# alex-petrenko/sample-factory

Measured on AMD Instinct MI355X. Metric: env-steps/sec (whole node), 4096 envs, 84x84x4 obs, higher is better.
Workload: dtype f32

## Files before the change

include/sf_hip.h:

```cpp
#ifndef SF_HIP_H
#define SF_HIP_H

#include <stdint.h>

#ifdef __cplusplus
extern "C" {
#endif

#define SF_OK 0
#define SF_ERR_ARG (-1)
#define SF_ERR_LAUNCH (-2)
#define SF_ERR_UNSUPPORTED (-3)
#define SF_MAX_ACTION_HEADS 64

const char *sf_last_error(void);
int sf_abi_version(void);

int sf_valid_mask(const int32_t *policy_id, const float *policy_version, uint8_t *valids, uint8_t *valids_flat,
                  float *actions, int num_actions, float *log_prob_actions, int E, int T, int my_policy_id,
                  int train_step, int max_policy_lag, int32_t *num_invalid, void *stream);

int sf_gae_returns(float *rewards, const uint8_t *dones, const uint8_t *time_outs, const float *values,
                   const uint8_t *valids, const double *rms_stats, int E, int T, float gamma, float gae_lambda,
                   int value_bootstrap, float *advantages, float *returns, void *stream);
// ... 35 lines not shown
    int32_t action_kind;
    int32_t dense_adv;
    int32_t num_heads;
    int32_t head_n[8];
    int32_t old_values_T;
} sf_loss_cfg;

int sf_ppo_loss(const float *params, int ld_params, const float *values, int ld_values, const float *actions,
                const float *old_logp, const float *old_params, const float *old_values, const float *adv,
                const float *targets, const uint8_t *valids, const int32_t *index, int64_t offset, int64_t n, int A,
                const sf_loss_cfg *h_cfg, const double *moments, double *sums, float *g_params, float *g_values,
                float *ratio_out ,
                void *stream);
int sf_ppo_loss_heads(const float *params, int ld_params, const float *values, int ld_values, const float *actions,
                      const float *old_logp, const float *old_params, const float *old_values, const float *adv,
                      const float *targets, const uint8_t *valids, const int32_t *index, int64_t offset, int64_t n, int A,
                      const sf_loss_cfg *h_cfg, const double *moments, double *sums, float *g_params, float *g_values,
                      float *ratio_out, const int32_t *head_n , int num_heads, void *stream);
int sf_ppo_loss_masked(const float *params, int ld_params, const float *values, int ld_values, const float *actions,
                       const float *old_logp, const float *old_params, const float *old_values, const float *adv,
                       const float *targets, const uint8_t *valids, const int32_t *index, int64_t offset, int64_t n, int A,
                       const sf_loss_cfg *h_cfg, const double *moments, double *sums, float *g_params, float *g_values,
                       float *ratio_out, const int32_t *head_n , int num_heads, const uint8_t *mask,
                       int64_t ld_mask, int mask_T, void *stream);
int sf_vtrace_masked(const float *params, int ld_params, const float *values, int ld_values, const float *actions,
                     const float *old_logp, const float *rewards, const uint8_t *dones, const int32_t *index,
                     int64_t offset, int64_t n, int A, int action_kind, int recurrence, float gamma, float rho_hat,
                     float c_hat, float *vs, float *adv, const int32_t *head_n , int num_heads,
                     const uint8_t *mask, int64_t ld_mask, int mask_T, void *stream);
int sf_consistency_loss(const float *params_t, const float *params_s, int ld_params, const float *values_t,
                        const float *values_s, int ld_values, const uint8_t *valids, const int32_t *index, int64_t offset,
                        int64_t n, int A, int action_kind, const int32_t *head_n , int num_heads,
                        float coeff_policy, float coeff_value, const double *moments, double *sums, float *g_params_s,
                        float *g_values_s, void *stream);
int sf_loss_scalars(const double *sums, const double *moments, const sf_loss_cfg *h_cfg, float *out, void *stream);
int sf_train_summaries(const uint8_t *valids, const float *ratio, const float *values, int ld_values,
                       const float *old_values, int old_values_T, const float *actions, int num_actions, const float *adv,
                       int dense_adv, const int32_t *policy_id, const float *policy_version, const float *action_logits,
                       int A, const int32_t *index, int64_t offset, int64_t n, int my_policy_id, int train_step,
                       float clip_ratio, const float *exp_avg_sq, int64_t P, double *out, void *stream);

int sf_minibatch_indices(int32_t *out, int64_t experience_size, int recurrence, int shuffle, uint32_t seed,
                         uint32_t epoch, void *stream);
int sf_minibatch_expand(const int32_t *chunk_starts, int32_t *out, int64_t experience_size, int recurrence,
                        void *stream);

int sf_grad_sumsq(const float *g, int64_t P, double *sumsq, void *stream);
int sf_adam_step(float *p, const float *g, float *m, float *v, int64_t P, int step, float lr, float beta1,
                 float beta2, float eps, float max_grad_norm, const double *sumsq, float grad_scale,
                 const uint32_t *skip_flag, void *stream);
int sf_adam_step_dlr(float *p, const float *g, float *m, float *v, int64_t P, int step, const float *lr_dev,
                     float lr_scale, float beta1, float beta2, float eps, float max_grad_norm, const double *sumsq,
                     float grad_scale, const uint32_t *skip_flag, void *stream);
int sf_lr_kl_adaptive(const float *kl, float *lr_dev, float threshold, float lr_min, float lr_max, float *lr_out,
                      void *stream);
int sf_clock_probe(unsigned long long *out, int spin_cycles, void *stream);

int sf_lamb_step(float *p, const float *g, float *m, float *v, float *scratch, const uint8_t *seg_id, double *seg_sums,
                 int64_t P, int num_segments, int step, float lr, float beta1, float beta2, float eps,
                 float weight_decay, float min_trust, float max_grad_norm, const double *sumsq, float grad_scale,
                 const uint32_t *skip_flag, void *stream);

int sf_sample_write_step(const float *logits, int ld_logits, const float *values, int ld_values, int B, int A, int T,
                         int t, uint32_t seed, uint32_t step, uint32_t row0, float policy_version, int deterministic,
                         int action_kind, float *traj_actions,
                         float *traj_logits, float *traj_logp, float *traj_values, float *traj_policy_version,
                         int32_t *env_actions, void *stream);

int sf_sample_write_step_masked(const float *logits, int ld_logits, const float *values, int ld_values,
                                const uint8_t *action_mask, int64_t ld_mask, int B, int A, int T, int t, uint32_t seed,
                                uint32_t step, uint32_t row0, float policy_version, int deterministic,
                                float *traj_actions, float *traj_logits, float *traj_logp, float *traj_values,
                                float *traj_policy_version, int32_t *env_actions, void *stream);

int sf_sample_write_step_tuple(const float *logits, int ld_logits, const float *values, int ld_values, int B,
                               int num_heads, const int32_t *head_n, int T, int t, uint32_t seed, uint32_t step,
                               uint32_t row0, float policy_version, int deterministic, float *traj_actions,
                               float *traj_logits, float *traj_logp, float *traj_values, float *traj_policy_version,
                               int32_t *env_actions, void *stream);

int sf_sample_write_step_tuple_masked(const float *logits, int ld_logits, const float *values, int ld_values,
                                      const uint8_t *action_mask, int64_t ld_mask, int B, int num_heads,
                                      const int32_t *head_n, int T, int t, uint32_t seed, uint32_t step, uint32_t row0,
                                      float policy_version, int deterministic, float *traj_actions, float *traj_logits,
                                      float *traj_logp, float *traj_values, float *traj_policy_version,
                                      int32_t *env_actions, void *stream);

int sf_traj_write_env_step(const float *rewards, const uint8_t *terminated, const uint8_t *truncated, int B, int T,
                           int t, float reward_scale, float reward_clip, int policy_id, float *traj_rewards,
                           uint8_t *traj_dones, uint8_t *traj_time_outs, int32_t *traj_policy_id, float *ep_return,
                           int32_t *ep_len, double *ep_stats, void *stream);

int sf_traj_write_env_step_active(const float *rewards, const uint8_t *terminated, const uint8_t *truncated, int B, int T,
                                  int t, float reward_scale, float reward_clip, int policy_id, float *traj_rewards,
                                  uint8_t *traj_dones, uint8_t *traj_time_outs, int32_t *traj_policy_id, float *ep_return,
                                  int32_t *ep_len, double *ep_stats, const uint8_t *active_in, uint8_t *active_state,
                                  void *stream);

int sf_synth_vec_step(float *state, const float *actions, int64_t act_stride, float *obs_out, int64_t out_stride, int B,
                      int D, int A, int env0, uint32_t seed, uint32_t step, int reset, float *rewards,
                      uint8_t *terminated, void *stream);

int sf_h2d_rows(void *dst, int64_t dst_pitch, const void *src, int64_t src_pitch, int64_t row_bytes, int64_t rows,
                void *stream);
int sf_copy_rows(void *dst, int64_t dst_pitch, const void *src, int64_t src_pitch, int64_t row_bytes, int64_t rows,
                 void *stream);
// ... 12 lines not shown
                 void *stream);
int sf_synth_step(const int32_t *actions, int B, int env0, int num_actions, uint32_t seed, uint32_t step,
                  float *rewards, uint8_t *terminated, void *stream);

int sf_pixcatch_state_words(int k);
int sf_pixcatch_reset(int32_t *state, uint8_t *obs_out, int64_t out_pitch, int N, int env0, uint32_t seed, int H, int W,
                      int k, int balls, void *stream);
int sf_pixcatch_step(int32_t *state, const int32_t *actions, uint8_t *obs_out, int64_t out_pitch, float *rewards,
                     uint8_t *terminated, int N, int env0, uint32_t seed, int H, int W, int k, int balls, void *stream);
int sf_pixcatch_reset_levels(int32_t *state, uint8_t *obs_out, int64_t out_pitch, int N, int env0, uint32_t seed, int H,
                             int W, int k, int balls, int decoys, int levels, uint32_t start_level, void *stream);
int sf_pixcatch_step_levels(int32_t *state, const int32_t *actions, uint8_t *obs_out, int64_t out_pitch, float *rewards,
                            uint8_t *terminated, int N, int env0, uint32_t seed, int H, int W, int k, int balls, int decoys,
                            int levels, uint32_t start_level, void *stream);

int sf_random_shift_gather(void *dst, int64_t dst_sample_pitch, const void *src, int64_t src_sample_pitch,
                           const int32_t *index, int64_t offset, int64_t n, int traj_T, int C, int H, int W, int elem_bytes,
                           int pad, int recurrence, uint32_t seed, uint32_t draw_id, void *stream);

typedef struct {
    int32_t Cin, H, W;
    int32_t Cout, KH, KW, stride;
    int32_t OH, OW;
    int32_t in_u8;
    int32_t relu;
    int32_t traj_T;
    float sub_mean, inv_scale;
} sf_conv_desc;

int64_t sf_conv_fwd_workspace(int64_t n, const sf_conv_desc *h_desc);
int sf_conv_fwd(const void *in, int64_t in_sample_stride, const int32_t *index, int64_t offset, const float *w,
                const float *bias, float *out, int64_t n, const sf_conv_desc *h_desc, void *workspace,
                int64_t workspace_bytes, void *stream);
int64_t sf_conv_wgrad_workspace(int64_t n, const sf_conv_desc *h_desc);
int sf_conv_wgrad(const void *in, int64_t in_sample_stride, const int32_t *index, int64_t offset, const float *dout,
                  float *dw, float *db, int64_t n, const sf_conv_desc *h_desc, void *workspace, void *stream);
int sf_conv_dgrad(const float *dout, const float *w, const float *in_act, float *din, int64_t n,
                  const sf_conv_desc *h_desc, void *stream);
int sf_conv_relu_mask_supported(int64_t n, const sf_conv_desc *h_desc);
int sf_conv_fwd_relu_mask(const void *in, int64_t in_sample_stride, const int32_t *index, int64_t offset, const float *w,
                          const float *bias, float *out, uint32_t *relu_mask, int64_t n, const sf_conv_desc *h_desc,
                          void *stream);
int sf_conv_wgrad_relu_mask(const void *in, int64_t in_sample_stride, const int32_t *index, int64_t offset,
                            const float *dout, const uint32_t *relu_mask, float *dw, float *db, int64_t n,
                            const sf_conv_desc *h_desc, void *workspace, void *stream);

int sf_conv_norm_supported(int64_t n, const sf_conv_desc *h_desc);
int sf_conv_fwd_norm(const void *in, int64_t in_sample_stride, const int32_t *index, int64_t offset, const float *mu,
                     const float *rstd, const float *w, const float *bias, float *out, int64_t n,
                     const sf_conv_desc *h_desc, void *stream);
int sf_conv_wgrad_norm(const void *in, int64_t in_sample_stride, const int32_t *index, int64_t offset, const float *mu,
                       const float *rstd, const float *dout, float *dw, float *db, int64_t n, const sf_conv_desc *h_desc,
                       void *workspace, void *stream);

int sf_mlp2_fwd(const float *x, int64_t x_stride, int64_t n, int D, float sub_mean, float inv_scale, const float *mu,
                const float *rstd, const float *w1, const float *b1, int H1, const float *w2, const float *b2, int H2,
                int act, float *out, void *stream);

int sf_rnn_store_state(const float *h, const float *c, const uint8_t *dones, int64_t done_stride, float *out,
                       int64_t out_stride, int64_t B, int H, void *stream);

int sf_rnn_store_state_held(const float *h, const float *c, const uint8_t *dones, int64_t done_stride, const float *prev,
                            int64_t prev_stride, const int32_t *policy_id, int64_t pid_stride, float *out,
                            int64_t out_stride, int64_t B, int H, void *stream);

int sf_rnn_chunk_setup(const uint8_t *dones, const uint8_t *valids, const float *rnn_states, const int32_t *index,
                       int64_t offset, int Cn, int R, int S, int traj_T, float *keep_tm, float *h0, void *stream);

int sf_lstm_seq_supported(int Cn, int H);
int sf_lstm_seq_fwd(const float *gx, const float *whh, const float *bhh, const float *keep, float *gates, float *hprev,
                    float *hout, float *cprev, float *cout, uint32_t *sync, int R, int Cn, int H, int env_major,
                    void *stream);
int sf_lstm_seq_bwd(const float *dout, const float *gates, const float *cprev, const float *cout, const float *keep,
                    const float *whh, float *dgx, uint32_t *sync, int R, int Cn, int H, int env_major, void *stream);

int sf_gru_seq_fwd(const float *gx, const float *whh, const float *bhh, const float *keep, float *gates, float *hprev,
                   float *hout, uint32_t *sync, int R, int Cn, int H, int env_major, void *stream);
int sf_gru_seq_bwd(const float *dout, const float *gates, const float *hprev, const float *keep, const float *whh,
                   float *dgx, float *dgh, uint32_t *sync, int R, int Cn, int H, int env_major, void *stream);

int sf_seq_fwd_x_supported(int Cn, int H, int Kx);
int sf_lstm_seq_fwd_x(const float *x, const float *wih_t, const float *bih, int Kx, const float *whh, const float *bhh,
                      const float *keep, float *gates, float *hprev, float *hout, float *cprev, float *cout,
                      uint32_t *sync, int R, int Cn, int H, int env_major, void *stream);
int sf_gru_seq_fwd_x(const float *x, const float *wih_t, const float *bih, int Kx, const float *whh, const float *bhh,
                     const float *keep, float *gates, float *hprev, float *hout, uint32_t *sync, int R, int Cn, int H,
                     int env_major, void *stream);

int sf_rnn_rowseq_supported(int kind, int Cn, int H);
int sf_rnn_rowseq_fwd(int kind, const float *gx, const float *whh, const float *bhh, const float *keep, float *gates,
                      float *hprev, float *hout, float *cprev, float *cout, int R, int Cn, int H, int env_major, void *stream);
int sf_rnn_rowseq_bwd(int kind, const float *dout, const float *gates, const float *hprev, const float *cprev,
                      const float *cout, const float *keep, const float *whh, float *dgx, float *dgh,
                      int R, int Cn, int H, int env_major, void *stream);

int sf_rnn_wideseq_supported(int kind, int Cn, int H);
int sf_rnn_seq_slab_rows(int kind, int H, int pass);
int sf_rnn_wideseq_fwd(int kind, const float *gx, const float *whh, const float *bhh, const float *keep, float *gates,
                       float *hprev, float *hout, float *cprev, float *cout, uint32_t *sync, int R, int Cn, int H,
                       int env_major, void *stream);
int sf_rnn_wideseq_bwd(int kind, const float *dout, const float *gates, const float *hprev, const float *cprev,
                       const float *cout, const float *keep, const float *whh, float *dgx, float *dgh, uint32_t *sync,
                       int R, int Cn, int H, int env_major, void *stream);

#define SF_DP_UNIQUE_ID_BYTES 128
int sf_dp_unique_id(void *out_id);
// ... 88 lines not shown
```

sample_factory_amd/algo/learning/learner.py:

```python
from __future__ import annotations

import glob
import time
import os
from os.path import join
from typing import Dict, List, Optional, Tuple

import numpy as np
import torch

from sample_factory_amd import lib
from sample_factory_amd.algo.learning.dp import ReplicaGroup
from sample_factory_amd.algo.utils.tensor_dict import TensorDict
from sample_factory_amd.cfg.arguments import augment_consistency_coeff
from sample_factory_amd.envs.frame_ops import random_shift_seed
from sample_factory_amd.envs.spaces import (action_head_sizes, calc_num_action_parameters, calc_num_actions, is_box,
                                             is_discrete)
from sample_factory_amd.model.actor_critic import ActorCritic
from sample_factory_amd.model.model_factory import create_actor_critic
from sample_factory_amd.utils.attr_dict import AttrDict
from sample_factory_amd.utils.decay import LinearDecay
from sample_factory_amd.utils.utils import log

LEARNER_ENV_STEPS, POLICY_ID_KEY, STATS_KEY, TRAIN_STATS = "learner_env_steps", "policy_id", "stats", "train"
# ... 308 lines not shown
        ac = self.actor_critic
        keep_p = ac.flat_params.clone()
        sd = dict(ref)
        ac.load_state_dict(sd, strict=False)
        flat.copy_(ac.flat_params)
        ac.flat_params.copy_(keep_p)
        ac.params_changed()

    def load_from_checkpoint(self, policy_id, load_progress=True) -> None:
        prefix = dict(latest="checkpoint", best="best")[self.cfg.load_checkpoint_kind]
        cps = self.get_checkpoints(self.checkpoint_dir(self.cfg, policy_id), pattern=f"{prefix}_*")
        cp = self.load_checkpoint(cps, self.device)
        if cp is not None:
            self._load_state(cp, load_progress)

    def set_new_cfg(self, new_cfg: Dict) -> None:
        self.new_cfg = new_cfg

    def set_policy_to_load(self, policy_to_load) -> None:
        self.policy_to_load = policy_to_load

    def _refresh_loss_cfg(self) -> None:
        cfg = self.cfg
        self.loss_cfg = lib.sf_loss_cfg(
            clip_ratio=cfg.ppo_clip_ratio, clip_value=cfg.ppo_clip_value, value_loss_coeff=cfg.value_loss_coeff,
            exploration_coeff=cfg.exploration_loss_coeff, kl_coeff=cfg.kl_loss_coeff,
            exploration_kind=0 if cfg.exploration_loss_coeff == 0.0 else (1 if cfg.exploration_loss == "entropy" else 2),
            action_kind=1 if is_box(self.env_info.action_space) else 0, dense_adv=int(bool(cfg.with_vtrace)))
        heads = action_head_sizes(self.env_info.action_space)
        self._head_sizes = heads
        if 1 < len(heads) <= len(self.loss_cfg.head_n):
            self.loss_cfg.num_heads = len(heads)
            for i, nh in enumerate(heads):
                self.loss_cfg.head_n[i] = nh

    def _maybe_update_cfg(self) -> None:
        if self.new_cfg is None:
            return
        for key, value in self.new_cfg.items():
            setattr(self.cfg, key, value)
        if self.cfg.lr_schedule == "constant" and self.curr_lr != self.cfg.learning_rate:
            self.curr_lr = self.cfg.learning_rate
        self._refresh_loss_cfg()
        self.new_cfg = None

    def _maybe_load_policy(self) -> None:
        if self.policy_to_load is None:
            return
        self.load_from_checkpoint(self.policy_to_load, load_progress=False)
        self.train_step += self.cfg.max_policy_lag + 1
        self.policy_versions_tensor[self.policy_id] = self.train_step
        self.policy_to_load = None

    def _prepare_batch(self, batch: TensorDict) -> Tuple[AttrDict, int, int]:
        cfg, ac = self.cfg, self.actor_critic
        multi = getattr(ac, "multi_key", False)
        obs = {k: batch["obs"][k] for k in ac.obs_keys} if multi else batch["obs"]["obs"]
        E, T = batch["rewards"].shape
        N = E * T
        valids_flat = ac._buf(("prep", "valids_flat"), (N,), dtype=torch.bool)
        lib.valid_mask(batch["policy_id"], batch["policy_version"], batch["valids"], batch["actions"],
                       self.num_actions, batch["log_prob_actions"], self.policy_id, self.train_step,
                       cfg.max_policy_lag, self._num_invalid, valids_flat=valids_flat)
        if not ac.training:
            ac.train()
        if ac.obs_normalizer is not None:
            ac.obs_normalizer.update(obs, ac.obs_elems, E * (T + 1))
        last = {k: v[:, T] for k, v in obs.items()} if multi else obs[:, T]
        rnn = dict(states=batch["rnn_states"][:, T]) if cfg.use_rnn else None
        heads = ac.forward_heads(last, E, sample_stride=0 if multi else obs.stride(0), tag="boot", rnn=rnn)[-1]
        lib.copy_rows(batch["values"][:, T], heads[:, 0])
        adv = torch.empty((E, T), dtype=torch.float32, device=self.device)
        ret = torch.empty((E, T), dtype=torch.float32, device=self.device)
        buff = AttrDict()
        if not cfg.with_vtrace:
            rms = ac.returns_normalizer.stats if cfg.normalize_returns else None
            lib.gae_returns(batch["rewards"], batch["dones"], batch["time_outs"], batch["values"], batch["valids"],
                            rms, cfg.gamma, cfg.gae_lambda, cfg.value_bootstrap, adv, ret)
            buff.advantages, buff.returns = adv.view(N), ret.view(N)
        elif cfg.value_bootstrap:
            lib.gae_returns(batch["rewards"], batch["dones"], batch["time_outs"], batch["values"], batch["valids"],
                            None, cfg.gamma, cfg.gae_lambda, True, adv, ret)
        buff.obs = obs
        buff.actions = batch["actions"].view(N, self.num_actions)
        buff.action_logits = batch["action_logits"].view(N, self.num_action_params)
        buff.log_prob_actions = batch["log_prob_actions"].view(N)
        buff.rewards = batch["rewards"].view(N)
        buff.dones = batch["dones"].view(N)
        buff.policy_id, buff.policy_version = batch["policy_id"].view(N), batch["policy_version"].view(N)
        if cfg.use_rnn:
            buff.rnn_states = batch["rnn_states"]
        buff["values"] = batch["values"]
        buff.valids = valids_flat
        buff.E, buff.T = E, T
        if getattr(self, "_loss_mask_on", False):
            buff.action_mask = batch["obs"]["action_mask"]
        if cfg.normalize_returns and not cfg.with_vtrace:
            ac.returns_normalizer(buff.returns)
        num_invalids = int(self._num_invalid.item())
        if self.dp:
            t = torch.tensor([num_invalids], dtype=torch.int64, device=self.device)
            self._all_reduce(t)
            self._global_invalids = int(t.item())
        else:
            self._global_invalids = num_invalids
        return buff, N, num_invalids

    def _get_minibatches(self, batch_size, experience_size):
        cfg = self.cfg
        assert cfg.rollout % cfg.recurrence == 0
        assert experience_size % batch_size == 0, f"experience size: {experience_size}, batch size: {batch_size}"
        n_mb = cfg.num_batches_per_epoch
        if n_mb == 1:
            return [(None, 0, experience_size)]
        assert n_mb * batch_size == experience_size, \
            f"dataset of {experience_size} samples != num_batches_per_epoch {n_mb} x batch_size {batch_size}"
        if cfg.shuffle_minibatches:
            idx = torch.empty(experience_size, dtype=torch.int32, device=self.device)
            if getattr(cfg, "device_shuffle", False):
                seed = (cfg.seed or 0) * 7919 + self.policy_id
                lib.minibatch_indices(idx, experience_size, cfg.recurrence, True, seed, self._shuffle_epoch)
                self._shuffle_epoch += 1
            else:
                starts = np.random.permutation(np.arange(0, experience_size, cfg.recurrence))
                starts_dev = torch.from_numpy(starts.astype(np.int32)).to(self.device, non_blocking=True)
                lib.minibatch_expand(starts_dev, idx, experience_size, cfg.recurrence)
            return [(idx[i * batch_size:(i + 1) * batch_size], 0, batch_size) for i in range(experience_size // batch_size)]
        return [(None, i * batch_size, batch_size) for i in range(n_mb)]

    _shuffle_epoch = 0

    def _calculate_losses(self, mb: AttrDict, num_invalids: int):
        from sample_factory_amd.algo.utils.action_distributions import get_action_distribution
        buff, part = (mb if isinstance(mb, tuple) else (mb, None))
        if part is None:
            part = (None, 0, buff.E * buff.T)
        acts, g_heads, sc = self._losses_native(buff, part, num_invalids)
        index, offset, n = part
        heads = acts[-1]
        A = self.num_action_params
        space = self.env_info.action_space
        rows = index.long() if index is not None else torch.arange(offset, offset + n, device=self.device)
        mask = buff.get("action_mask")
        mrows = None if mask is None else mask[:, :buff.T].reshape(buff.E * buff.T, -1)[rows]
        dist = get_action_distribution(space, heads[:n, 1:1 + A], mrows)
        dist.raw_logits, dist.values = heads[:n, 1:1 + A], heads[:n, 0]
        kl_old = dist.kl_divergence(get_action_distribution(space, buff.action_logits[rows], mrows))[buff.valids[rows]]
        summaries = AttrDict(adv_mean=sc[6], adv_std=sc[7], num_valid=sc[8], entropy=sc[9], kl_divergence_max=sc[5],
                             kl_old_mean=sc[4].clone(), ratio=self._ratio[:n], values=heads[:n, 0], g_heads=g_heads)
        return dist, sc[0].clone(), sc[1].clone(), kl_old, sc[2].clone(), sc[3].clone(), summaries

    def _losses_native(self, buff: AttrDict, mb, num_invalids: int, scalars_out: Optional[torch.Tensor] = None,
                       moments: Optional[torch.Tensor] = None, first_of: Optional[Tuple[int, int]] = None):
        cfg, ac = self.cfg, self.actor_critic
        index, offset, n = mb
        A = self.num_action_params
        alpha = getattr(self, "_cons_coeff", 0.0) if getattr(self, "_shift_pad", 0) > 0 else 0.0
        m = 2 * n if alpha > 0.0 else n
        rnn = None
# ... 37 lines not shown
            vs = ac._buf(("vt", "vs"), (n,))
            adv = ac._buf(("vt", "adv"), (n,))
            lib.vtrace(params, ld, values, ld, buff.actions, buff.log_prob_actions, buff.rewards, buff.dones, index,
                       offset, n, A, self.loss_cfg.action_kind, cfg.recurrence, cfg.gamma, cfg.vtrace_rho,
                       cfg.vtrace_c, vs, adv, head_sizes=self._head_sizes, **mkw)
            lib.moments(adv, buff.valids, index, n, self._moments, offset=offset, dense_x=True)
            adv_arr, tgt_arr = adv, vs
        elif moments is None:
            lib.moments(buff.advantages, buff.valids, index, n, self._moments, offset=offset)
            adv_arr, tgt_arr = buff.advantages, buff.returns
        else:
            adv_arr, tgt_arr = buff.advantages, buff.returns
        if moments is None:
            moments = self._moments
            self._all_reduce(moments)
        self._ratio = ac._buf(("loss", "ratio"), (n,))
        self.loss_cfg.old_values_T = buff.T
        lib.ppo_loss(params, ld, values, ld, buff.actions, buff.log_prob_actions, buff.action_logits, buff["values"],
                     adv_arr, tgt_arr, buff.valids, index, offset, n, A, self.loss_cfg, moments, self._sums,
                     g_heads[:n, 1:], g_heads[:n, 0], ratio_out=self._ratio, head_sizes=self._head_sizes, **mkw)
        if m > n:
            if not hasattr(self, "_cons_sums"):
                self._cons_sums = torch.zeros(4, dtype=torch.float64, device=self.device)
            lib.consistency_loss(params, heads[n:, 1:], ld, values, heads[n:, 0], ld, buff.valids, index, offset, n, A,
                                 self.loss_cfg.action_kind, alpha, alpha, moments, self._cons_sums, g_heads[n:, 1:],
                                 g_heads[n:, 0], head_sizes=self._head_sizes)
        self._last_mb = (index, offset, n, values, adv_arr)
        if self.dp and self._dp_reduce_each_mb:
            self.group.loss_sums(self._sums)
        out = scalars_out if scalars_out is not None else torch.zeros(16, dtype=torch.float32, device=self.device)
        lib.loss_scalars(self._sums, moments, self.loss_cfg, out)
        if m > n:
            c = self._cons_sums
            nv = c[3].clamp(min=1.0)
            out[11:14].copy_(torch.stack((c[0] / nv, c[2], c[1] / nv)))
        return acts, g_heads, out

    def _epoch_moments(self, buff: AttrDict, minibatches) -> Optional[torch.Tensor]:
        if not self.dp or self.cfg.with_vtrace or not getattr(self.cfg, "dp_epoch_moments", True):
            return None
        tab = self.actor_critic._buf(("loss", "epoch_moments"), (len(minibatches), 3), dtype=torch.float64)
        for i, (index, offset, n) in enumerate(minibatches):
            lib.moments(buff.advantages, buff.valids, index, n, tab[i], offset=offset)
        self._all_reduce(tab)
        return tab

    def _train(self, buff: AttrDict, batch_size: int, experience_size: int, num_invalids: int) -> Optional[AttrDict]:
        cfg, ac = self.cfg, self.actor_critic
        early_stopping_tolerance = 1e-6
        prev_epoch_actor_loss = 1e9
        recent_kls: List[float] = []
        num_sgd_steps = 0
        n_mb = cfg.num_batches_per_epoch
        self._scalars = ac._buf(("loss", "scalars"), (cfg.num_epochs * n_mb, 16))
        global_size = experience_size * self.world
        need_kl_each_mb = self.lr_scheduler.invoke_after_each_minibatch() and isinstance(self.lr_scheduler, KlAdaptiveScheduler)
        self._dp_reduce_each_mb = need_kl_each_mb
        lr_on_device = need_kl_each_mb and cfg.optimizer == "adam"
        if lr_on_device:
            if not hasattr(self, "_lr_dev"):
                self._lr_dev = torch.zeros(1, dtype=torch.float32, device=self.device)
            self._lr_dev.fill_(float(self.curr_lr))
        self._grad_norms = []
        skip = ac.rnn_abort_word() if hasattr(ac, "rnn_abort_word") else None
        if skip is not None:
            ac.rnn_abort_clear()
        for epoch in range(cfg.num_epochs):
            minibatches = self._get_minibatches(batch_size, experience_size)
            mom_tab = self._epoch_moments(buff, minibatches)
            for batch_num, mb in enumerate(minibatches):
                row = self._scalars[epoch * n_mb + batch_num]
                acts, g_heads, _ = self._losses_native(buff, mb, num_invalids, row,
                                                       moments=None if mom_tab is None else mom_tab[batch_num],
                                                       first_of=(epoch, batch_num))
                index, offset, n = mb
                if self._dp_split is not None:
                    cut = ac._segs[self._dp_split][0]
                    pending = []
                    ac.backward(acts, g_heads, self._mb_frames[0], self._mb_rows, sample_stride=ac.obs_elems,
                                **self._mb_frames[1],
                                on_layer_done=lambda li: pending.append(self.group.all_reduce_grads_async(
                                    ac.flat_grads[cut:])) if li == self._dp_split else None)
                    self.group.all_reduce_grads(ac.flat_grads[:cut])
                    for work in pending:
                        work.wait()
                else:
                    ac.backward(acts, g_heads, self._mb_frames[0], self._mb_rows, sample_stride=ac.obs_elems,
                                **self._mb_frames[1])
                    if self.dp:
                        self.group.all_reduce_grads(ac.flat_grads)
                actual_lr = self.curr_lr
                valid_frac = 1.0
                if self._global_invalids > 0:
                    valid_frac = (global_size - self._global_invalids) / global_size
                    actual_lr = self.curr_lr * valid_frac
                self.adam_step_count += 1
                use_clip = cfg.max_grad_norm > 0.0
                if use_clip or getattr(cfg, "record_grad_norm", False):
                    lib.grad_sumsq(ac.flat_grads, self._sumsq)
                    if getattr(cfg, "record_grad_norm", False):
                        self._grad_norms.append(float(self._sumsq.sqrt().item()))
                if cfg.optimizer == "lamb":
                    if self._lamb is None:
                        seg, nseg = ac.tensor_segment_ids()
                        self._lamb = (seg, nseg, torch.empty_like(ac.flat_params),
                                      torch.zeros(128, dtype=torch.float64, device=self.device))
                    seg, nseg, scratch, seg_sums = self._lamb
                    lib.lamb_step(ac.flat_params, ac.flat_grads, self.exp_avg, self.exp_avg_sq, scratch, seg, seg_sums,
                                  nseg, self.adam_step_count, actual_lr, cfg.adam_beta1, cfg.adam_beta2, cfg.adam_eps,
                                  1e-4, 0.01, cfg.max_grad_norm if use_clip else 0.0, self._sumsq if use_clip else None,
                                  skip_flag=skip)
                elif lr_on_device:
                    lib.adam_step_dlr(ac.flat_params, ac.flat_grads, self.exp_avg, self.exp_avg_sq, self.adam_step_count,
                                      self._lr_dev, valid_frac, cfg.adam_beta1, cfg.adam_beta2, cfg.adam_eps,
                                      cfg.max_grad_norm if use_clip else 0.0, self._sumsq if use_clip else None,
                                      skip_flag=skip)
                else:
                    lib.adam_step(ac.flat_params, ac.flat_grads, self.exp_avg, self.exp_avg_sq, self.adam_step_count,
                                  actual_lr, cfg.adam_beta1, cfg.adam_beta2, cfg.adam_eps,
                                  cfg.max_grad_norm if use_clip else 0.0, self._sumsq if use_clip else None,
                                  skip_flag=skip)
                ac.params_changed()
                num_sgd_steps += 1
                self.train_step += 1
                if lr_on_device:
                    sch = self.lr_scheduler
                    lib.lr_kl_adaptive(row[4:5], self._lr_dev, sch.threshold, sch.min_lr, sch.max_lr, lr_out=row[10:11])
                elif need_kl_each_mb:
                    recent_kls.append(float(row[4].item()))
                    self.curr_lr = self.lr_scheduler.update(self.curr_lr, recent_kls)
                elif self.lr_scheduler.invoke_after_each_minibatch():
                    self.curr_lr = self.lr_scheduler.update(self.curr_lr, recent_kls)
                self.policy_versions_tensor[self.policy_id] = self.train_step
            blk = self._scalars[epoch * n_mb:(epoch + 1) * n_mb]
            if self.dp and not need_kl_each_mb:
                flag = (skip.to(torch.float32) if skip is not None else blk.new_zeros(1)).expand(blk.shape[0], 1)
                pack = torch.cat([blk[:, [0, 1, 2, 3, 4, 9, 5]], flag], dim=1).contiguous()
                self.group.reduce_sum_max(pack, (6, 7))
                blk[:, [0, 1, 2, 3, 4, 9, 5]] = pack[:, :7]
                aborted = skip is not None and bool(pack[0, 7].item() != 0)
            elif self.dp and skip is not None:
                aborted = bool(self.group.all_reduce_max(skip.to(torch.float32)).item() != 0)
            else:
                aborted = skip is not None and ac.rnn_pass_aborted()
            rows = blk.cpu()
            if aborted:
                raise lib.SfHipError(
                    "a fused recurrent sequence pass was aborted (a work-group never arrived: is the GPU shared with "
                    "another process?); the optimiser steps after it were skipped, the weights are those of the last "
                    "good SGD step; set SF_LSTM_SEQ=0 to use the per-step kernels")
            actor_losses = (rows[:, 0] + rows[:, 1] + rows[:, 2]).double().numpy()
            if lr_on_device:
                self.curr_lr = float(rows[-1, 10])
                actual_lr = self.curr_lr * valid_frac
            if not need_kl_each_mb or lr_on_device:
                recent_kls.extend(rows[:, 4].double().tolist())
            if self.lr_scheduler.invoke_after_each_epoch():
                self.curr_lr = self.lr_scheduler.update(self.curr_lr, recent_kls)
            new_epoch_actor_loss = float(np.mean(actor_losses))
            if abs(prev_epoch_actor_loss - new_epoch_actor_loss) < early_stopping_tolerance:
                break
            prev_epoch_actor_loss = new_epoch_actor_loss
        last = rows[-1]
        stats = AttrDict(lr=self.curr_lr, actual_lr=actual_lr, env_steps=self.env_steps,
                         policy_loss=float(last[0]), exploration_loss=float(last[1]),
                         kl_loss=float(last[2]), value_loss=float(last[3]), kl_divergence=float(last[4]),
                         kl_divergence_max=float(last[5]), adv_mean=float(last[6]), adv_std=float(last[7]),
                         entropy=float(last[9]), loss=float(last[0] + last[1] + last[2] + last[3]),
                         num_sgd_steps=num_sgd_steps)
        if getattr(self, "_cons_coeff", 0.0) > 0.0:
            stats.update(consistency_kl=float(last[11]), consistency_kl_max=float(last[12]),
                         consistency_value=float(last[13]))
        if self._should_save_summaries():
            stats.update(self._record_summaries(buff))
            self._last_summary_time = time.time()
        self.last_summary = stats
        return stats

    _last_summary_time = 0.0
    _summary_rate_decay = LinearDecay([(0, 2.0), (100000, 60.0), (1000000, 120.0)])

    def _should_save_summaries(self) -> bool:
        every = self._summary_rate_decay.at(float(self.train_step))
        return time.time() - self._last_summary_time >= every or getattr(self.cfg, "summaries_every_train", False)

    def _record_summaries(self, buff: AttrDict) -> Dict[str, float]:
        index, offset, n, values, adv_arr = self._last_mb
        if not hasattr(self, "_summ"):
            self._summ = torch.empty(24, dtype=torch.float64, device=self.device)
        ld = values.stride(0) if values.dim() == 1 else 1
        lib.train_summaries(buff.valids, self._ratio, values, ld, buff["values"], buff.T, buff.actions, self.num_actions,
                            adv_arr, bool(self.cfg.with_vtrace), buff.policy_id, buff.policy_version, buff.action_logits,
                            self.num_action_params, index, offset, n, self.policy_id, self.train_step,
                            self.loss_cfg.clip_ratio, self.exp_avg_sq, self._summ)
        o = self._summ.cpu().tolist()
        rows, nv, ns = o[0], o[1], o[2]
        has_v, has_s = nv > 0, ns > 0
        return dict(
            valids_fraction=nv / rows, same_policy_fraction=ns / rows, value=o[3] / rows,
            ratio_mean=o[4] / nv if has_v else 0.0, ratio_min=o[8] if has_v else 1.0, ratio_max=o[9] if has_v else 1.0,
            fraction_clipped=o[5] / nv if has_v else 0.0, value_delta=o[6] / rows, value_delta_max=o[10],
            act_min=o[11], act_max=o[12], adv_min=o[13], adv_max=o[14], max_abs_logprob=o[15],
            version_diff_avg=o[7] / ns if has_s else 0.0, version_diff_min=o[16] if has_s else 0.0,
            version_diff_max=o[17] if has_s else 0.0, grad_norm=float(self._sumsq.sqrt().item()),
            adam_max_second_moment=o[18])

    def train(self, batch: TensorDict) -> Optional[Dict]:
        self._maybe_update_cfg()
        self._maybe_load_policy()
        buff, experience_size, num_invalids = self._prepare_batch(batch)
        if self._global_invalids >= experience_size * self.world:
            return None
        train_stats = self._train(buff, self.cfg.batch_size, experience_size, num_invalids)
        frameskip = self.env_info.frameskip if self.cfg.summaries_use_frameskip else 1
        self.env_steps += experience_size * self.world * frameskip
        stats = {LEARNER_ENV_STEPS: self.env_steps, POLICY_ID_KEY: self.policy_id}
        if train_stats is not None:
            stats[TRAIN_STATS] = train_stats
        return stats
```

sample_factory_amd/csrc/sf_nn.hip:

```cpp
#include "sf_common.h"
#include <stdarg.h>
#include <stdlib.h>
#include <string.h>
#ifndef SF_GLDS_ABLATE
#define SF_GLDS_ABLATE 0
#endif
#include <type_traits>
#include <algorithm>

#define STREAM(s) reinterpret_cast<hipStream_t>(s)

typedef float f32x16 __attribute__((ext_vector_type(16)));

extern "C" int sf_selftest_host(void) {
    const uint32_t ds[] = {1, 2, 3, 4, 6, 7, 9, 20, 32, 33, 49, 64, 81, 84, 128, 400, 512, 576, 3136, 7056, 28224, 65535, 1000003};
    for (uint32_t d : ds) {
        const FastDiv f = make_fastdiv(d);
        const uint32_t ns[] = {0, 1, d - 1, d, d + 1, 2 * d - 1, 2 * d, 12345678, 0x7FFFFFFFu, 0x7FFFFFFFu - d, 13107200, 13107199};
        for (uint32_t n : ns) if (fdiv(n, f) != n / d) return -1;
        for (uint32_t n = 0; n < 200000; n += 7) if (fdiv(n, f) != n / d) return -2;
        for (uint32_t n = 0x7FFFFFFFu; n > 0x7FFFFFFFu - 100000; n -= 13) if (fdiv(n, f) != n / d) return -3;
    }
    const uint32_t areas[] = {1, 2, 3, 35, 70, 96, 485, 5760, 19200, 33600, 76800, 921600, 8388607, 8388608};
    for (uint32_t D : areas) {
// ... 554 lines not shown
                const int64_t base = patch_base(m, mok, po);
                if constexpr (MODE == MODE_F32)
                    ra[s].v = *reinterpret_cast<const float4 *>(reinterpret_cast<const float *>(in) + base + tapo[s]);
                else
                    ra[s] = load_act_raw<MODE_GENERIC>(g, in, base, po, (uint32_t)(k0row + kg[s]), aok[s]);
            }
        }
#pragma unroll
        for (int s = 0; s < T::SB; ++s) {
            const int64_t m = mc + bkk0 + s * BROWS;
            bok[s] = m < mend;
            rb[s] = load_row_raw<VECB>(dy, bok[s] ? m : mbeg, n0 + bcg, N);
        }
    };
    const bool do_colsum = partial_b != nullptr && blockIdx.x == 0 && tid < BN;
    float colacc = 0.f;
    if (mbeg < mend) gload(mbeg);
    for (int64_t mc = mbeg; mc < mend; mc += 32) {
        __syncthreads();
#pragma unroll
        for (int s = 0; s < T::SA; ++s) {
            const int lrow = FR ? (tid & 31) : (tid >> 5) + 8 * s;
            *reinterpret_cast<float4 *>(&As[lrow * LDA + kg[s]]) =
                act_finish<MODE>(g, ra[s], MODE != MODE_GENERIC || aok[s]);
        }
        const bool tail = mc + 32 > mend;
#pragma unroll
        for (int s = 0; s < T::SB; ++s)
            *reinterpret_cast<float4 *>(&Bs[(bkk0 + s * BROWS) * LDB + bcg]) =
                (VECB && !tail) ? rb[s] : row_finish(rb[s], bok[s], n0 + bcg, N);
        __syncthreads();
        if (mc + 32 < mend) gload(mc + 32);
        if (do_colsum) {
#pragma unroll 8
            for (int kk = 0; kk < 32; ++kk) colacc += Bs[kk * LDB + tid];
        }
        mma_chunk<T::TM, T::TN, LDA, LDB>(As, Bs, wm * T::TM * 32, wn * T::TN * 32, lane, acc);
    }
    if (do_colsum && n0 + tid < N) partial_b[(int64_t)blockIdx.z * N + n0 + tid] = colacc;
    float *dst = partial + (int64_t)blockIdx.z * K * N;
#pragma unroll
    for (int tm = 0; tm < T::TM; ++tm)
#pragma unroll
        for (int tn = 0; tn < T::TN; ++tn) {
            const int n = n0 + wn * T::TN * 32 + tn * 32 + (lane & 31);
#pragma unroll
            for (int r = 0; r < 16; ++r) {
                const int k = k0row + wm * T::TM * 32 + tm * 32 + FRAG_ROW(r, lane);
                if (k < K && n < N) dst[(int64_t)k * N + n] = acc[tm][tn][r];
            }
        }
}

__global__ __launch_bounds__(256) void k_reduce_partials(const float *__restrict__ partial, float *__restrict__ out,
                                                         int64_t n, int Z) {
    for (int64_t i = (int64_t)blockIdx.x * blockDim.x + threadIdx.x; i < n; i += (int64_t)gridDim.x * blockDim.x) {
        float s[8] = {0.f, 0.f, 0.f, 0.f, 0.f, 0.f, 0.f, 0.f};
        int z = 0;
        for (; z + 8 <= Z; z += 8) {
#pragma unroll
            for (int j = 0; j < 8; ++j) s[j] += partial[(int64_t)(z + j) * n + i];
        }
        for (int j = 0; z < Z; ++z, ++j) s[j] += partial[(int64_t)z * n + i];
        out[i] = ((s[0] + s[1]) + (s[2] + s[3])) + ((s[4] + s[5]) + (s[6] + s[7]));
    }
}

__global__ __launch_bounds__(256) void k_reduce_partials_tree(const float *__restrict__ partial, float *__restrict__ out,
                                                              int64_t n, int Z) {
    __shared__ float sm[8][33];
    const int li = threadIdx.x & 31, zg = threadIdx.x >> 5;
    const int64_t i = (int64_t)blockIdx.x * 32 + li;
    const int zper = (Z + 7) / 8, z0 = zg * zper, z1 = z0 + zper < Z ? z0 + zper : Z;
    float s[8] = {0.f, 0.f, 0.f, 0.f, 0.f, 0.f, 0.f, 0.f};
    if (i < n) {
        int z = z0;
        for (; z + 8 <= z1; z += 8) {
#pragma unroll
            for (int j = 0; j < 8; ++j) s[j] += partial[(int64_t)(z + j) * n + i];
        }
        for (int j = 0; z < z1; ++z, ++j) s[j] += partial[(int64_t)z * n + i];
    }
    sm[zg][li] = ((s[0] + s[1]) + (s[2] + s[3])) + ((s[4] + s[5]) + (s[6] + s[7]));
    __syncthreads();
    if (zg == 0 && i < n)
        out[i] = ((sm[0][li] + sm[1][li]) + (sm[2][li] + sm[3][li])) + ((sm[4][li] + sm[5][li]) + (sm[6][li] + sm[7][li]));
}
#define SF_SWITCHES(X)                                                                                                  \
    X(reduce_tree, "SF_REDUCE_TREE", 1) X(conv1_bf16, "SF_CONV1_BF16", 1) X(conv1_img, "SF_CONV1_IMG", 1)              \
    X(conv1_wgs, "SF_CONV1_WGS", 2) X(conv1_wide, "SF_CONV1_WIDE", 1) X(conv1_norm, "SF_CONV1_NORM", 1)                \
    X(relu_mask, "SF_RELU_MASK", 1) X(fwd_img, "SF_FWD_IMG", 1) X(linear_narrow, "SF_LINEAR_NARROW", 1)                \
    X(linear_dual, "SF_LINEAR_DUAL", 1) X(glds_cfg, "SF_GLDS_CFG", 0) X(glds_splitk, "SF_GLDS_SPLITK", 1)              \
    X(glds_fc64, "SF_GLDS_FC64", 1) X(glds_wide_min, "SF_GLDS_WIDE_MIN", 384) X(glds_min_tiles, "SF_GLDS_MIN_TILES", 768) \
    X(glds_small64, "SF_GLDS_SMALL64", 256) X(glds_force64, "SF_GLDS_FORCE64", 0) X(glds_split64, "SF_GLDS_SPLIT64", 32) \
    X(glds_zl, "SF_GLDS_ZL", 2) X(glds_tailsplit, "SF_GLDS_TAILSPLIT", 1) X(glds_tall, "SF_GLDS_TALL", 0)              \
    X(glds_persist, "SF_GLDS_PERSIST", 0) X(xcd_raster, "SF_XCD_RASTER", 1) X(xcd_rows, "SF_XCD_ROWS", 0)              \
    X(tap_perm, "SF_TAP_PERM", 0) X(wgrad_glds, "SF_WGRAD_GLDS", 1) X(wgrad_glds_min, "SF_WGRAD_GLDS_MIN", -1)         \
    X(wgrad_glds_k64, "SF_WGRAD_GLDS_K64", 1) X(wgrad_img, "SF_WGRAD_IMG", 3) X(wgrad_zl, "SF_WGRAD_ZL", 1)            \
    X(dgrad_linear, "SF_DGRAD_LINEAR", 1) X(dgrad_linear64, "SF_DGRAD_LINEAR64", 1) X(dgrad_lpt, "SF_DGRAD_LPT", 1)    \
    X(dgrad_zl, "SF_DGRAD_ZL", 3) X(dgrad_pix, "SF_DGRAD_PIX", 1) X(debug_occ, "SF_DEBUG_OCC", 0)
struct Switches {
#define X(field, name, dflt) int64_t field;
    SF_SWITCHES(X)
#undef X
    bool debug_img;
};
static int64_t env_num(const char *name, int64_t dflt) {
    const char *v = getenv(name);
    return v ? atoll(v) : dflt;
}
static Switches read_switches() {
    Switches s;
#define X(field, name, dflt) s.field = env_num(name, dflt);
    SF_SWITCHES(X)
#undef X
    s.debug_img = getenv("SF_DEBUG_IMG") != nullptr;
    return s;
}
static const Switches &sw() {
    static const Switches s = read_switches();
    return s;
}

static void launch_reduce_partials(const float *partial, float *out, int64_t n, int Z, hipStream_t st) {
    if (sw().reduce_tree && Z >= 64 && (n + 255) / 256 < 256)
        k_reduce_partials_tree<<<dim3((unsigned)((n + 31) / 32)), dim3(256), 0, st>>>(partial, out, n, Z);
    else
        k_reduce_partials<<<dim3((unsigned)((n + 255) / 256 < 2048 ? (n + 255) / 256 : 2048)), dim3(256), 0, st>>>(partial, out, n, Z);
}

template <int BM, int BN, int WM, int WN, bool VEC>
__global__ __launch_bounds__(256) void k_conv_dgrad(ConvG g, const float *__restrict__ dy,
                                                    const float *__restrict__ w, const float *__restrict__ in_act,
                                                    float *__restrict__ din, int64_t nsamples) {
    using T = Tile<BM, BN, WM, WN>;
    constexpr int LDA = BM + 1, LDB = BN + 1;
    __shared__ __attribute__((aligned(16))) float As[32 * LDA];
    __shared__ __attribute__((aligned(16))) float Bs[32 * LDB];
    const int tid = threadIdx.x, lane = tid & 63, wave = tid >> 6;
    const int wm = wave / WN, wn = wave % WN;
    const int ph = blockIdx.z / g.S, pw = blockIdx.z % g.S;
    const int Hc = (g.H - ph + g.S - 1) / g.S, Wc = (g.W - pw + g.S - 1) / g.S;
    const int KHs = (g.KH - ph + g.S - 1) / g.S, KWs = (g.KW - pw + g.S - 1) / g.S;
    const int64_t Mc = nsamples * Hc * Wc;
    const int64_t m0 = (int64_t)blockIdx.x * BM;
    if (m0 >= Mc || Hc <= 0 || Wc <= 0) return;
    const int n0 = blockIdx.y * BN;
    const int Cin = g.Cin, Cout = g.Cout;
    const int Kp = KHs * KWs * Cout;

    const int kq = (tid & 7) * 4;
    const FastDiv fHW = g.dHcWc[blockIdx.z], fW = g.dWc[blockIdx.z], fKWs = g.dKWs[blockIdx.z];
    int arow[T::SA], aih[T::SA], aiw[T::SA];
    bool aval[T::SA];
    const uint32_t HcWc = (uint32_t)(Hc * Wc);
#pragma unroll
    for (int s = 0; s < T::SA; ++s) {
        const int64_t m = m0 + (tid >> 3) + 32 * s;
        aval[s] = m < Mc;
        const uint32_t mm = aval[s] ? (uint32_t)m : 0u;
        const uint32_t smp = fdiv(mm, fHW), pix = mm - smp * HcWc;
        aih[s] = (int)fdiv(pix, fW);
        aiw[s] = (int)pix - aih[s] * Wc;
        arow[s] = (int)(smp * (uint32_t)(g.OH * g.OW)) + aih[s] * g.OW + aiw[s];
    }
    const bool kfull = (Kp & 31) == 0;
    f32x16 acc[T::TM][T::TN];
    ZERO_ACC(acc);

    float4 ra[T::SA], rb[T::SB];
    bool aok[T::SA], bok = true;
    int ncol = 0;
    auto gload = [&](int k0) {
        const int k = k0 + kq;
        const bool kval = k < Kp;
        const int kc = kval ? k : 0;
        const int tap = (int)fdiv((uint32_t)kc, g.dCout);
        const int n = kc - tap * Cout;
        ncol = n;
        const int a = (int)fdiv((uint32_t)tap, fKWs), b = tap - a * KWs;
        const int drow = a * g.OW + b;
// ... 687 lines not shown
extern "C" int sf_conv_fwd_t_os2(const float *in, int64_t in_sample_stride, const float *in2, const float *wt, const float *bias,
                                 float *out, int64_t out_sample_stride, float *out2, int64_t keep_n, int64_t n,
                                 const sf_conv_desc *h_desc, void *stream) {
    return conv_fwd_t_os_impl("sf_conv_fwd_t_os2", in, in_sample_stride, in2, wt, bias, out, out_sample_stride, out2, keep_n, n,
                              h_desc, stream);
}
static int conv_fwd_os_supported_impl(int op, int64_t n, int64_t keep_n, const sf_conv_desc *h_desc, int64_t in_sample_stride,
                                      int64_t out_sample_stride) {
    if (!h_desc || n <= 0 || keep_n < 0 || keep_n > n || check_desc(h_desc, "sf_conv_fwd_os_supported") != 0 ||
        in_sample_stride % 4 != 0 || !out_stride_ok(h_desc, nullptr, out_sample_stride) ||
        n * (int64_t)h_desc->OH * h_desc->OW >= (1LL << 31))
        return 0;
    if (op == 0) {
        if (!relu_mask_ok(h_desc, n)) return 0;
        Operands o = query_operands(h_desc, false);
        o.stride = in_sample_stride;
        return plan_conv_fwd(h_desc, make_geom(h_desc), n, o).kernel == K_CONV1_U8_BF16_W ? 1 : 0;
    }
    if (op != 3) return 0;
    const ConvPlan p = plan_conv_fwd_t(h_desc, n, in_sample_stride, nullptr, true, keep_n);
    return (p.kernel == K_FWD_IMG || p.kernel == K_FWD_GLDS_ZT || p.kernel == K_FWD_GLDS_Z) && p.splits == 1 ? 1 : 0;
}
extern "C" int sf_conv_fwd_os_supported(int op, int64_t n, const sf_conv_desc *h_desc, int64_t in_sample_stride,
                                        int64_t out_sample_stride) {
    return conv_fwd_os_supported_impl(op, n, n, h_desc, in_sample_stride, out_sample_stride);
}
extern "C" int sf_conv_fwd_os2_supported(int op, int64_t n, int64_t keep_n, const sf_conv_desc *h_desc, int64_t in_sample_stride,
                                         int64_t out_sample_stride) {
    return conv_fwd_os_supported_impl(op, n, keep_n, h_desc, in_sample_stride, out_sample_stride);
}

extern "C" int sf_linear_fwd_dual_supported(int64_t n, int N, int K1, int K2) {
    return sw().linear_dual && n > 0 && N >= 64 && K1 > 0 && K2 > 0 && K1 % 32 == 0 && K2 % 32 == 0 && n < (1LL << 31) &&
           cdiv64(n, 128) * (int64_t)cdiv64(N, 64) >= 256;
}
extern "C" int sf_linear_fwd_dual(const float *a1, int64_t lda1, const float *w1t, const float *bias1, int K1,
                                  const float *a2, int64_t lda2, const float *w2t, const float *bias2, int K2, float *out,
                                  int64_t n, int N, int gru_H, void *stream) {
    SF_REQUIRE(a1 && w1t && a2 && w2t && out && n > 0 && N > 0, "sf_linear_fwd_dual: bad args");
    SF_REQUIRE(K1 > 0 && K2 > 0 && K1 % 32 == 0 && K2 % 32 == 0 && lda1 % 4 == 0 && lda2 % 4 == 0 && n < (1LL << 31),
               "sf_linear_fwd_dual: K1, K2 must be multiples of 32 and the row strides multiples of 4 (K1=%d K2=%d)", K1, K2);
    SF_REQUIRE((((uintptr_t)a1 | (uintptr_t)a2 | (uintptr_t)w1t | (uintptr_t)w2t) & 15) == 0,
               "sf_linear_fwd_dual: operands must be 16-byte aligned");
    SF_REQUIRE(gru_H == 0 || (gru_H > 0 && gru_H % 64 == 0 && N == 4 * gru_H),
               "sf_linear_fwd_dual: the GRU column layout needs N == 4 * gru_H and gru_H %% 64 == 0 (N=%d gru_H=%d)", N, gru_H);
    k_fwd_glds2<128, 64, 2, 2><<<dim3(cdiv64(n, 128), cdiv64(N, 64)), dim3(256), 0, STREAM(stream)>>>(
        a1, lda1, w1t, bias1, K1, a2, lda2, w2t, bias2, K2, out, n, N, gru_H);
    return sf_launch_status("sf_linear_fwd_dual");
}
extern "C" int sf_transpose(const float *w, float *wt, int K, int N, void *stream) {
    SF_REQUIRE(w && wt && K > 0 && N > 0, "sf_transpose: bad args");
    k_transpose<<<dim3(cdiv64(K, 32), cdiv64(N, 32)), dim3(256), 0, STREAM(stream)>>>(w, wt, K, N);
    return sf_launch_status("sf_transpose");
}

struct SplitPlan {
    int Z;
    int64_t m_per_split;
};
static SplitPlan plan_splits(int64_t Mtot, int K, int N, int BM, int BN, int bpc = 0) {
    const int64_t tiles = (int64_t)((K + BM - 1) / BM) * ((N + BN - 1) / BN);
    const int64_t chunks = (Mtot + 31) / 32;
    int64_t zcap = (2304 + tiles - 1) / tiles;
    const int64_t zmax = (chunks + 7) / 8;
    if (zcap > zmax) zcap = zmax;
    if (zcap < 1) zcap = 1;
    if (zcap > 1024) zcap = 1024;
    int64_t Z = zcap;
    if (bpc > 0) {
        const double slots = 256.0 * bpc;
        double best = -1.0;
        for (int64_t z = 1; z <= zcap; ++z) {
            const double u = (double)(tiles * z) / slots, rounds = u <= 1.0 ? 1.0 : (double)(int64_t)(u + 0.999999);
            double eff = u / rounds;
            if (tiles * z < 256) eff *= 0.5;
            if (eff > best + 0.02) { best = eff; Z = z; }
        }
    }
    SplitPlan p;
    p.m_per_split = ((chunks + Z - 1) / Z) * 32;
    p.Z = (int)((Mtot + p.m_per_split - 1) / p.m_per_split);
    return p;
}
template <int BK, int BN, int WM, int WN>
static int occ_wgrad_glds() {
    static const int v = occupancy_of(k_wgrad_glds<BK, BN, WM, WN>);
    return v;
}
static inline int wgrad_bn(int N) { return N <= 32 ? 32 : 64; }
static int wgrad_ws_partials(int64_t Mtot, int K, int N) { return plan_splits(Mtot, K, N, 128, wgrad_bn(N)).Z; }
struct WgradGlds {
    int cfg;
    int BK, BN, Z;
    int64_t m_per_split;
};
static WgradGlds plan_wgrad_glds(int64_t Mtot, int K, int N, bool query_occupancy = false) {
    WgradGlds q;
    const bool k256 = K >= 256 && (K + 255) / 256 * 256 <= (K + 127) / 128 * 128;
    q.cfg = N >= 128 ? 1 : (k256 ? 0 : 2);
    if (sw().wgrad_glds >= 2) q.cfg = sw().wgrad_glds - 2;
    if (K == 64 && N >= 128) q.cfg = 3;
    q.BK = q.cfg == 0 ? 256 : q.cfg == 3 ? 64 : 128;
    q.BN = (q.cfg == 1 || q.cfg == 3) ? 128 : 64;
    int bpc = 0;
    if (query_occupancy)
        bpc = q.cfg == 0 ? occ_wgrad_glds<256, 64, 4, 1>() : q.cfg == 1 ? occ_wgrad_glds<128, 128, 2, 2>()
// ... 69 lines not shown
        plan_raster(p, sw().xcd_raster && p.grid.x * p.grid.y > 1);
        const bool zl = sw().wgrad_zl && g.KH == 1 && g.KW == 1 && g.H == 1 && g.W == 1 && g.OH == 1 && g.OW == 1 &&
                        n * o.stride < (1LL << 30) && Mtot * N < (1LL << 30);
        const TileArgs t = {q.BK, q.BN, q.cfg == 0 ? 4 : 2, q.cfg == 0 ? 1 : 2};
        if (zl) plan_tile(p, K_WGRAD_GLDS_Z, "k_wgrad_glds_z", t);
        else plan_tile(p, K_WGRAD_GLDS, "k_wgrad_glds", t);
        return p;
    } else {
        const int bpc = BN == 32 ? occ_wgrad_mode<32, 4, 1>(mode) : occ_wgrad_mode<64, 2, 2>(mode);
        const SplitPlan s = plan_splits(Mtot, K, N, 128, BN, bpc);
        p.variant = mode; p.partials = p.splits = s.Z; p.per_split = s.m_per_split;
        p.grid = dim3(cdiv64(K, 128), cdiv64(N, BN), (unsigned)s.Z);
        p.t = BN == 32 ? TileArgs{128, 32, 4, 1} : TileArgs{128, 64, 2, 2};
        plan_kernel(p, K_CONV_WGRAD, "k_conv_wgrad<%d, %d, %d, %d>", BN, p.t.WM, p.t.WN, mode);
        return p;
    }
    p.grid = dim3((unsigned)p.partials);
    return p;
}

extern "C" int64_t sf_conv_wgrad_workspace(int64_t n, const sf_conv_desc *h_desc) {
    if (!h_desc || n <= 0) return 0;
    const int K = h_desc->KH * h_desc->KW * h_desc->Cin, N = h_desc->Cout;
    const int64_t Mtot = n * h_desc->OH * h_desc->OW;
    int Z = wgrad_ws_partials(Mtot, K, N);
    if (wgrad_img_variant(h_desc, n) && wgrad_img_blocks(h_desc, n) > Z) Z = wgrad_img_blocks(h_desc, n);
    if (small_linear_wgrad_ok(h_desc)) {
        const int64_t zs = cdiv64(Mtot, 64) < 1024 ? cdiv64(Mtot, 64) : 1024;
        if (zs > Z) Z = (int)zs;
    }
    if (h_desc->in_u8 == IN_F32_NHWC) {
        const WgradGlds q = plan_wgrad_glds(Mtot, K, N);
        if (q.Z > Z) Z = q.Z;
    }
    return (int64_t)sizeof(float) * Z * ((int64_t)K * N + N) + 256;
}

#define WGRAD_LAUNCH(BN, WM, WN, MODE)                                                                                  \
    k_conv_wgrad<BN, WM, WN, MODE><<<p.grid, p.block, 0, st>>>(g, in, in_sample_stride, index, offset, dout, partial_w, \
                                                               partial_b, Mtot, p.per_split)
#define WGRAD_GLDS_ARGS g, inf, in_sample_stride, dout, partial_w, partial_b, Mtot, p.per_split, p.rx, p.ry, p.rtot
#define WGRAD_GLDS(BK_, BN_, WM_, WN_)                                                                                    \
    do {                                                                                                                  \
        if (p.kernel == K_WGRAD_GLDS_Z) k_wgrad_glds_z<BK_, BN_, WM_, WN_><<<p.grid, p.block, 0, st>>>(WGRAD_GLDS_ARGS);  \
        else k_wgrad_glds<BK_, BN_, WM_, WN_><<<p.grid, p.block, 0, st>>>(WGRAD_GLDS_ARGS);                               \
    } while (0)
#define WGRAD_STRIP(KERN, ...)                                                                                  \
    KERN<<<p.grid, p.block, p.lds, st>>>(g, reinterpret_cast<const uint8_t *>(in), in_sample_stride, index, offset, dout, \
                                         ##__VA_ARGS__, partial_w, partial_b, (int)n, (int)((n + 1) / 2))

static int conv_wgrad_impl(const void *in, int64_t in_sample_stride, const int32_t *index, int64_t offset,
                           const float *dout, const uint32_t *dmask, float *dw, float *db, int64_t n,
                           const sf_conv_desc *h_desc, void *workspace, void *stream, const float *mu = nullptr,
                           const float *rstd = nullptr) {
    int rc = check_desc(h_desc, "sf_conv_wgrad");
    if (rc) return rc;
    SF_REQUIRE(in && dout && dw && workspace && n > 0, "sf_conv_wgrad: bad args");
    SF_REQUIRE(((uintptr_t)workspace & 15) == 0, "sf_conv_wgrad: workspace must be 16-byte aligned");
    ConvG g = make_geom(h_desc);
    g.nmu = mu; g.nrstd = rstd;
    const int64_t Mtot = n * g.OH * g.OW;
    SF_REQUIRE(Mtot < (1LL << 31), "sf_conv_wgrad: M=%lld exceeds 2^31 rows; split the batch", (long long)Mtot);
    const int K = g.K, N = g.Cout;
    const ConvPlan p = plan_conv_wgrad(h_desc, g, n, Operands{in, in_sample_stride, index != nullptr, nullptr, dout, nullptr, 0});
    SF_REQUIRE(!dmask || p.kernel == K_CONV1_WGRAD_BF16,
               "sf_conv_wgrad_relu_mask: this launch does not resolve to the mask-consuming kernel");
    float *partial_w = reinterpret_cast<float *>(workspace);
    float *partial_b = db ? partial_w + (int64_t)p.partials * K * N : nullptr;
    hipStream_t st = STREAM(stream);
    const float *inf = reinterpret_cast<const float *>(in);
    switch (p.kernel) {
        case K_CONV1_WGRAD_BF16:
            if (p.variant) WGRAD_STRIP(k_conv1_wgrad_bf16<true>, dmask); else WGRAD_STRIP(k_conv1_wgrad_bf16<false>, dmask);
            break;
        case K_CONV1_WGRAD_IMG:
            if (p.variant) WGRAD_STRIP((k_conv1_wgrad_img<2, 4, true>)); else WGRAD_STRIP((k_conv1_wgrad_img<2, 4, false>));
            break;
        case K_LINEAR_WGRAD_SMALL:
            k_linear_wgrad_small<<<p.grid, p.block, 0, st>>>(inf, in_sample_stride, dout, partial_w, partial_b, Mtot, p.per_split, K, N);
            break;
        case K_WGRAD_IMG:
            if (p.variant == 1) k_wgrad_img<64, 9, 9, 3, 1, 1><<<p.grid, p.block, 0, st>>>(inf, in_sample_stride, dout, partial_w, partial_b, (int)n);
            else k_wgrad_img<32, 20, 20, 4, 2, 2><<<p.grid, p.block, 0, st>>>(inf, in_sample_stride, dout, partial_w, partial_b, (int)n);
            break;
        case K_WGRAD_GLDS:
        case K_WGRAD_GLDS_Z:
            if (TILE_IS(64, 128)) WGRAD_GLDS(64, 128, 2, 2);
            else if (TILE_IS(256, 64)) WGRAD_GLDS(256, 64, 4, 1);
            else if (TILE_IS(128, 128)) WGRAD_GLDS(128, 128, 2, 2);
            else WGRAD_GLDS(128, 64, 2, 2);
            break;
        default:
            if (TILE_IS(128, 32)) { BY_MODE(WGRAD_LAUNCH, 32, 4, 1) }
            else { BY_MODE(WGRAD_LAUNCH, 64, 2, 2) }
    }
    launch_reduce_partials(partial_w, dw, (int64_t)K * N, p.partials, st);
    if (db) launch_reduce_partials(partial_b, db, N, p.partials, st);
    return sf_launch_status("sf_conv_wgrad");
}

extern "C" int sf_conv_wgrad(const void *in, int64_t in_sample_stride, const int32_t *index, int64_t offset,
                             const float *dout, float *dw, float *db, int64_t n, const sf_conv_desc *h_desc,
                             void *workspace, void *stream) {
    return conv_wgrad_impl(in, in_sample_stride, index, offset, dout, nullptr, dw, db, n, h_desc, workspace, stream);
}
extern "C" int sf_conv_wgrad_relu_mask(const void *in, int64_t in_sample_stride, const int32_t *index, int64_t offset,
                                       const float *dout, const uint32_t *relu_mask, float *dw, float *db, int64_t n,
                                       const sf_conv_desc *h_desc, void *workspace, void *stream) {
    SF_REQUIRE(relu_mask && ((uintptr_t)relu_mask & 7) == 0, "sf_conv_wgrad_relu_mask: relu_mask must be an 8-byte aligned device buffer");
    SF_REQUIRE(h_desc && n > 0 && relu_mask_ok(h_desc, n) && ((uintptr_t)in & 3) == 0 && in_sample_stride % 4 == 0 &&
                   ((uintptr_t)dout & 15) == 0,
               "sf_conv_wgrad_relu_mask: unsupported layer / launch (see sf_conv_relu_mask_supported)");
    return conv_wgrad_impl(in, in_sample_stride, index, offset, dout, relu_mask, dw, db, n, h_desc, workspace, stream);
}

extern "C" int sf_conv_norm_supported(int64_t n, const sf_conv_desc *h_desc) {
    return h_desc && check_desc(h_desc, "sf_conv_norm_supported") == 0 && conv_norm_ok(h_desc, n) ? 1 : 0;
}
extern "C" int sf_conv_fwd_norm(const void *in, int64_t in_sample_stride, const int32_t *index, int64_t offset,
                                const float *mu, const float *rstd, const float *w, const float *bias, float *out,
                                int64_t n, const sf_conv_desc *h_desc, void *stream) {
    int rc = check_desc(h_desc, "sf_conv_fwd_norm");
    if (rc) return rc;
    SF_REQUIRE(in && mu && rstd && w && out && n > 0, "sf_conv_fwd_norm: bad args");
    SF_REQUIRE(conv_norm_ok(h_desc, n) && ((uintptr_t)mu & 3) == 0 && ((uintptr_t)rstd & 3) == 0 &&
                   (in_is_u8(h_desc->in_u8) || ((uintptr_t)in & 3) == 0),
               "sf_conv_fwd_norm: unsupported launch (see sf_conv_norm_supported; f32 frames and tables 4-byte aligned)");
    ConvG g = make_geom(h_desc);
    g.nmu = mu; g.nrstd = rstd;
    const ConvPlan p = plan_conv_fwd(h_desc, g, n, Operands{in, in_sample_stride, index != nullptr, w, nullptr, out, 0});
    if (p.kernel != K_CONV_U8_IMG_NORM)
        return conv_fwd_impl(in, in_sample_stride, index, offset, w, bias, out, nullptr, n, h_desc, nullptr, 0, stream, mu,
                             rstd);
    SF_REQUIRE(n * g.OH * g.OW < (1LL << 31), "sf_conv_fwd_norm: M exceeds 2^31 rows; split the batch");
    k_conv_u8_img_norm<2, 4, 5, 16><<<p.grid, p.block, p.lds, STREAM(stream)>>>(
        g, reinterpret_cast<const uint8_t *>(in), in_sample_stride, index, offset, w, bias, out, (int)n);
    return sf_launch_status("sf_conv_fwd_norm");
}
extern "C" int sf_conv_wgrad_norm(const void *in, int64_t in_sample_stride, const int32_t *index, int64_t offset,
                                  const float *mu, const float *rstd, const float *dout, float *dw, float *db, int64_t n,
                                  const sf_conv_desc *h_desc, void *workspace, void *stream) {
    int rc = check_desc(h_desc, "sf_conv_wgrad_norm");
    if (rc) return rc;
    SF_REQUIRE(in && mu && rstd && dout && dw && workspace && n > 0, "sf_conv_wgrad_norm: bad args");
    SF_REQUIRE(conv_norm_ok(h_desc, n) && ((uintptr_t)mu & 3) == 0 && ((uintptr_t)rstd & 3) == 0 &&
                   (in_is_u8(h_desc->in_u8) || ((uintptr_t)in & 3) == 0),
               "sf_conv_wgrad_norm: unsupported launch (see sf_conv_norm_supported; f32 frames and tables 4-byte aligned)");
    ConvG g = make_geom(h_desc);
    g.nmu = mu; g.nrstd = rstd;
    const ConvPlan p = plan_conv_wgrad(h_desc, g, n, Operands{in, in_sample_stride, index != nullptr, nullptr, dout, nullptr, 0});
    if (p.kernel != K_CONV1_WGRAD_IMG_NORM)
        return conv_wgrad_impl(in, in_sample_stride, index, offset, dout, nullptr, dw, db, n, h_desc, workspace, stream, mu,
                               rstd);
    SF_REQUIRE(((uintptr_t)workspace & 15) == 0, "sf_conv_wgrad_norm: workspace must be 16-byte aligned");
    const int K = g.K, N = g.Cout;
    float *partial_w = reinterpret_cast<float *>(workspace), *partial_b = db ? partial_w + (int64_t)p.partials * K * N : nullptr;
    hipStream_t st = STREAM(stream);
    WGRAD_STRIP((k_conv1_wgrad_img_norm<2, 4>));
    launch_reduce_partials(partial_w, dw, (int64_t)K * N, p.partials, st);
    if (db) launch_reduce_partials(partial_b, db, N, p.partials, st);
    return sf_launch_status("sf_conv_wgrad_norm");
}

static sf_conv_desc linear_desc(int K, int N, int relu);
static bool linear_dgrad_glds_ok(const ConvG &g, int64_t n) {
    return g.H == 1 && g.W == 1 && g.KH == 1 && g.KW == 1 && g.Cout % 32 == 0 && g.Cin >= 128 &&
           cdiv64(n, 128) * (int64_t)cdiv64(g.Cin, 128) >= 512;
}
static bool linear_dgrad_glds64_ok(const ConvG &g, int64_t n) {
    return sw().dgrad_linear64 && g.H == 1 && g.W == 1 && g.KH == 1 && g.KW == 1 && g.Cout % 32 == 0 && g.Cout >= 512 &&
           g.Cin == 64 && n >= 8192;
}
static bool dgrad_pix_zl(const ConvG &g, int64_t n) {
    return (sw().dgrad_zl & 2) && g.Cout % 64 == 0 && n * (int64_t)g.OH * g.OW * g.Cout < (1LL << 30) &&
           (int64_t)g.K * g.Cout < (1LL << 30);
}
static bool dgrad_quadrow_zl(const ConvG &g, int64_t n) {
    return (sw().dgrad_zl & 1) && g.Cout % 64 == 0 && n * (int64_t)g.OH * g.OW * g.Cout < (1LL << 30) &&
           (int64_t)g.K * g.Cout < (1LL << 30) && n * (int64_t)g.H * g.W * g.Cin < (1LL << 30);
}
static unsigned plan_quadrow_classes(QuadrowClasses &q, const ConvG &g, int64_t n, int BM) {
    const int Wg = g.W / g.S, KWs = g.KW / g.S;
    q.ncls = 0;
    q.n = (uint32_t)n;
    for (int iwc = 0; iwc < Wg; ++iwc) {
        const int lo = std::max(0, iwc - g.OW + 1), nb = std::max(0, std::min(KWs - 1, iwc) - lo + 1);
        QuadrowClass *last = q.ncls ? &q.c[q.ncls - 1] : nullptr;
        if (last && last->nb == nb && (nb == 0 || last->b_lo == lo)) { ++last->dw.d; continue; }
        QuadrowClass &c = q.c[q.ncls++];
        c.col0 = iwc; c.b_lo = lo; c.nb = nb; c.dw.d = 1;
    }
    std::stable_sort(q.c, q.c + q.ncls, [](const QuadrowClass &a, const QuadrowClass &b) {
        return a.nb != b.nb ? a.nb > b.nb : a.dw.d > b.dw.d;
    });
    unsigned tiles = 0;
    for (int i = 0; i < q.ncls; ++i) {
        q.c[i].tile0 = tiles;
        tiles += cdiv64(n * (int64_t)q.c[i].dw.d, BM);
        q.c[i].dw = make_fastdiv(q.c[i].dw.d);
    }
    return tiles;
}
static ConvPlan plan_conv_dgrad(const ConvG &g, int64_t n, const Operands &o) {
    ConvPlan p = plan_init();
    const bool al16 = aligned(o.dout, 16) && aligned(o.w, 16), vec = g.vecB && al16;
    p.per_split = (g.Cout + 31) / 32 * 32;
    const bool zl_fits = n * (int64_t)g.Cout < (1LL << 30) && (int64_t)g.Cin * g.Cout < (1LL << 30);
    if (sw().dgrad_linear && linear_dgrad_glds_ok(g, n) && al16) {
        p.grid = dim3(cdiv64(n, 128), cdiv64(g.Cin, 128), 1);
        plan_raster(p, sw().xcd_raster >= 2 && p.grid.y > 1);
        if (sw().glds_zl >= 2 && zl_fits) plan_tile(p, K_FWD_GLDS_Z, "k_fwd_glds_z", TileArgs{128, 128, 2, 2});
        else plan_tile(p, K_FWD_GLDS, "k_fwd_glds", TileArgs{128, 128, 2, 2}, ", 2");
        return p;
    }
// ... 157 lines not shown
```

sample_factory_amd/csrc/sf_nn_glds.h:

```cpp
#pragma once

#ifndef SF_GLDS_ABLATE
#define SF_GLDS_ABLATE 0
#endif
#define GLDS16(gsrc, ldst)                                                                       \
    __builtin_amdgcn_global_load_lds((const __attribute__((address_space(1))) void *)(gsrc),    \
                                     (__attribute__((address_space(3))) void *)(ldst), 16, 0, 0)

#define BARRIER_NOFENCE()                  \
    do {                                   \
        asm volatile("" ::: "memory");     \
        __builtin_amdgcn_s_barrier();      \
        asm volatile("" ::: "memory");     \
    } while (0)

template <int TM, int TN>
__device__ __forceinline__ void mma_chunk_rows(const float *__restrict__ As, const float *__restrict__ Bs, int arow0,
                                               int brow0, int lane, f32x16 (&acc)[TM][TN]) {
    const int r = lane & 31, h = lane >> 5, sw = (r >> 1) & 7;
    const float *ap = As + (arow0 + r) * 32, *bp = Bs + (brow0 + r) * 32;
#pragma unroll
    for (int c = 0; c < 4; ++c) {
        const int pos = (((2 * c + h) ^ sw) << 2);
        float4 a[TM], b[TN];
// ... 611 lines not shown
        const int row = (i * 4 + wave) * 8 + lrow;
        int n = n0 + row;
        n = n < N ? n : N - 1;
        const int sw = (lpos ^ ((row >> 1) & 7)) << 2;
        bs1[i] = w1t + (int64_t)(use1 ? n : 0) * K1 + sw;
        bs2[i] = w2t + (int64_t)(use2 ? n + row2_off : 0) * K2 + sw - K1;
    }
    f32x16 acc[TM][TN];
#pragma unroll
    for (int a_ = 0; a_ < TM; ++a_)
#pragma unroll
        for (int b_ = 0; b_ < TN; ++b_)
#pragma unroll
            for (int r_ = 0; r_ < 16; ++r_) acc[a_][b_][r_] = 0.f;
    auto issue = [&](int k0, int stage) {
        float *sa = lds + stage * STAGE, *sb = sa + BM * 32;
        const bool first = k0 < K1;
#pragma unroll
        for (int i = 0; i < AI; ++i) GLDS16((first ? as1[i] : as2[i]) + k0, sa + (i * 4 + wave) * 256);
#pragma unroll
        for (int i = 0; i < BI; ++i) GLDS16((first ? bs1[i] : bs2[i]) + k0, sb + (i * 4 + wave) * 256);
    };
    issue(kbeg, 0);
    int stage = 0, k0 = kbeg;
    for (; k0 + 32 < K; k0 += 32, stage ^= 1) {
        asm volatile("s_waitcnt vmcnt(0)" ::: "memory");
        BARRIER_NOFENCE();
        issue(k0 + 32, stage ^ 1);
        const float *sa = lds + stage * STAGE;
        mma_chunk_rows<TM, TN>(sa, sa + BM * 32, wm * TM * 32, wn * TN * 32, lane, acc);
    }
    asm volatile("s_waitcnt vmcnt(0)" ::: "memory");
    BARRIER_NOFENCE();
    {
        const float *sa = lds + stage * STAGE;
        mma_chunk_rows<TM, TN>(sa, sa + BM * 32, wm * TM * 32, wn * TN * 32, lane, acc);
    }
    const int lcol = lane & 31;
#pragma unroll
    for (int tn = 0; tn < TN; ++tn) {
        const int col = n0 + wn * TN * 32 + tn * 32 + lcol;
        if (col >= N) continue;
        const float b1 = (bias1 && use1) ? bias1[col] : 0.f, b2 = (bias2 && use2) ? bias2[col + row2_off] : 0.f;
#pragma unroll
        for (int tm = 0; tm < TM; ++tm)
#pragma unroll
            for (int r = 0; r < 16; ++r) {
                const int64_t row = m0 + wm * TM * 32 + tm * 32 + FRAG_ROW(r, lane);
                if (row < Mtot) out[row * N + col] = (acc[tm][tn][r] + b1) + b2;
            }
    }
}

__global__ __launch_bounds__(256) void k_transpose(const float *__restrict__ w, float *__restrict__ wt, int K, int N) {
    __shared__ float t[32][33];
    const int k0 = blockIdx.x * 32, n0 = blockIdx.y * 32, tx = threadIdx.x & 31, ty = threadIdx.x >> 5;
#pragma unroll
    for (int i = 0; i < 32; i += 8) {
        const int k = k0 + ty + i, n = n0 + tx;
        t[ty + i][tx] = (k < K && n < N) ? w[(int64_t)k * N + n] : 0.f;
    }
    __syncthreads();
#pragma unroll
    for (int i = 0; i < 32; i += 8) {
        const int n = n0 + ty + i, k = k0 + tx;
        if (n < N && k < K) wt[(int64_t)n * K + k] = t[tx][ty + i];
    }
}

__device__ __attribute__((aligned(128))) const float sf_zero_page[32] = {};

template <int BM, int BN, int WM, int WN, bool ZL>
__device__ __forceinline__ void dgrad_pix_body(ConvG g, const float *__restrict__ dy, const float *__restrict__ w,
                                               const float *__restrict__ in_act, float *__restrict__ din,
                                               int nsamples, int ntiles, int tiles8, int lpt) {
    constexpr int TM = BM / WM / 32, TN = BN / WN / 32;
    constexpr int AI = BM / 32, BI = BN / 32;
    constexpr int STAGE = (BM + BN) * 32;
    static_assert(WM * WN == 4 && TM >= 1 && TN >= 1 && BI >= 1, "4 waves per block");
    __shared__ __attribute__((aligned(1024))) float lds[2 * STAGE];
    const int tid = threadIdx.x, lane = tid & 63, wave = __builtin_amdgcn_readfirstlane(tid >> 6);
    const int wm = wave / WN, wn = wave % WN;
    const int Cin = g.Cin, Cout = g.Cout, S = g.S, OH = g.OH, OW = g.OW;
    const uint32_t xcd = blockIdx.x & 7u, local = blockIdx.x >> 3;
    uint32_t t;
    int ih;
    if (lpt) {
        const uint32_t per_rank = gridDim.x / (8u * (uint32_t)g.H), rank = local / per_rank;
        t = local - rank * per_rank;
        const int c = (g.H - 1) >> 1, d = (int)((rank + 1u) >> 1);
        ih = (rank & 1u) ? c + d : c - d;
    } else {
        ih = (int)(local % (uint32_t)g.H);
        t = local / (uint32_t)g.H;
    }
    const int st = (int)((t % (uint32_t)tiles8) * 8u + xcd), ct = (int)(t / (uint32_t)tiles8);
    if (st >= ntiles) return;
    const int s0 = st * BM, n0 = ct * BN;
    const int CC = Cout >> 5;

    const int lrow = lane >> 3, lpos = lane & 7;
    const float *asrc[AI], *bsrc[BI];
#pragma unroll
    for (int i = 0; i < AI; ++i) {
        const int row = (i * 4 + wave) * 8 + lrow;
        int s = s0 + row;
        s = s < nsamples ? s : nsamples - 1;
        asrc[i] = dy + (int64_t)s * (OH * OW) * Cout + ((lpos ^ ((row >> 1) & 7)) << 2);
    }
#pragma unroll
    for (int i = 0; i < BI; ++i) {
        const int row = (i * 4 + wave) * 8 + lrow;
        int c = n0 + row;
        c = c < Cin ? c : Cin - 1;
        bsrc[i] = w + (int64_t)c * Cout + ((lpos ^ ((row >> 1) & 7)) << 2);
    }
    const int ph = ih % S, ihc = ih / S, KHs = (g.KH - ph + S - 1) / S;
    const int a_lo = ihc - OH + 1 > 0 ? ihc - OH + 1 : 0, a_hi = ihc < KHs - 1 ? ihc : KHs - 1;

    f32x16 acc[TM][TN];
// ... 1162 lines not shown
```

sample_factory_amd/csrc/sf_rl.hip:

```cpp
#include "sf_common.h"

thread_local char sf_err_buf[512] = "";

extern "C" const char *sf_last_error(void) { return sf_err_buf; }
extern "C" int sf_abi_version(void) { return 19; }

#define STREAM(s) reinterpret_cast<hipStream_t>(s)

__device__ __forceinline__ float clampf(float x, float lo, float hi) { return fminf(fmaxf(x, lo), hi); }

__global__ __launch_bounds__(256) void k_valid_mask(const int32_t *__restrict__ policy_id,
                                                    const float *__restrict__ policy_version,
                                                    uint8_t *__restrict__ valids, uint8_t *__restrict__ valids_flat,
                                                    float *__restrict__ actions,
                                                    int num_actions, float *__restrict__ logp, int E, int T,
                                                    int my_pid, int train_step, int max_lag,
                                                    int32_t *__restrict__ num_invalid) {
    const int64_t i = (int64_t)blockIdx.x * blockDim.x + threadIdx.x;
    const int64_t N = (int64_t)E * T;
    const bool in = i < N;
    bool valid = true;
    if (in) {
        const int64_t e = i / T;
        const int t = (int)(i - e * T);
// ... 1956 lines not shown
    return sf_launch_status("sf_minibatch_indices");
}

extern "C" int sf_minibatch_expand(const int32_t *chunk_starts, int32_t *out, int64_t experience_size, int recurrence,
                                   void *stream) {
    SF_REQUIRE(chunk_starts && out && experience_size > 0 && recurrence > 0 && experience_size % recurrence == 0,
               "sf_minibatch_expand: experience_size=%lld recurrence=%d", (long long)experience_size, recurrence);
    SF_REQUIRE(experience_size < (1LL << 31), "sf_minibatch_expand: experience too large for int32 indices");
    const int64_t n_chunks = experience_size / recurrence;
    k_minibatch_indices<<<dim3((unsigned)((n_chunks + 255) / 256)), dim3(256), 0, STREAM(stream)>>>(
        out, n_chunks, recurrence, 0, 0, 0u, chunk_starts);
    return sf_launch_status("sf_minibatch_expand");
}

__global__ __launch_bounds__(256) void k_grad_sumsq(const float *__restrict__ g, int64_t P,
                                                    double *__restrict__ sumsq) {
    __shared__ double lds[4];
    double acc[1] = {0.0};
    const int64_t nvec = P / 4;
    const float4 *g4 = reinterpret_cast<const float4 *>(g);
    const int64_t tid = (int64_t)blockIdx.x * blockDim.x + threadIdx.x, nt = (int64_t)gridDim.x * blockDim.x;
    for (int64_t i = tid; i < nvec; i += nt) {
        const float4 v = g4[i];
        acc[0] += (double)v.x * v.x + (double)v.y * v.y + (double)v.z * v.z + (double)v.w * v.w;
    }
    for (int64_t i = nvec * 4 + tid; i < P; i += nt) acc[0] += (double)g[i] * g[i];
    sf_block_sum<1>(acc, lds);
    if (threadIdx.x == 0) atomicAdd(sumsq, acc[0]);
}

extern "C" int sf_grad_sumsq(const float *g, int64_t P, double *sumsq, void *stream) {
    SF_REQUIRE(g && sumsq && P > 0, "sf_grad_sumsq: bad args");
    SF_REQUIRE(((uintptr_t)g & 15) == 0, "sf_grad_sumsq: gradient buffer must be 16-byte aligned");
    int rc = sf_hip_status(hipMemsetAsync(sumsq, 0, sizeof(double), STREAM(stream)), "sf_grad_sumsq memset");
    if (rc) return rc;
    const int64_t blocks = (P / 4 + 255) / 256;
    k_grad_sumsq<<<dim3((unsigned)(blocks < 1024 ? (blocks ? blocks : 1) : 1024)), dim3(256), 0, STREAM(stream)>>>(
        g, P, sumsq);
    return sf_launch_status("sf_grad_sumsq");
}

struct AdamC {
    float lr_step, bc2_sqrt, w1, b2, w2, eps, max_norm, grad_scale;
};

__device__ __forceinline__ void adam1(float &p, float g, float &m, float &v, const AdamC &c, float coef) {
    g = g * coef;
    m = m + (g - m) * c.w1;
    v = v * c.b2 + (g * g) * c.w2;
    const float denom = sqrtf(v) / c.bc2_sqrt + c.eps;
    p = p - c.lr_step * (m / denom);
}

__global__ __launch_bounds__(256) void k_adam(float *__restrict__ p, const float *__restrict__ g,
                                              float *__restrict__ m, float *__restrict__ v, int64_t P, AdamC c,
                                              const double *__restrict__ sumsq, const uint32_t *__restrict__ skip,
                                              const float *__restrict__ lr_dev) {
    if (skip && *skip) return;
    if (lr_dev) c.lr_step *= *lr_dev;
    float coef = c.grad_scale;
    if (sumsq && c.max_norm > 0.f) {
        const float total = (float)sqrt(*sumsq) * fabsf(c.grad_scale);
        const float cc = c.max_norm / (total + 1e-6f);
        coef = c.grad_scale * fminf(cc, 1.0f);
    }
    const int64_t nvec = P / 4;
    const int64_t tid = (int64_t)blockIdx.x * blockDim.x + threadIdx.x, nt = (int64_t)gridDim.x * blockDim.x;
    float4 *p4 = reinterpret_cast<float4 *>(p), *m4 = reinterpret_cast<float4 *>(m), *v4 = reinterpret_cast<float4 *>(v);
    const float4 *g4 = reinterpret_cast<const float4 *>(g);
    for (int64_t i = tid; i < nvec; i += nt) {
        float4 pp = p4[i], mm = m4[i], vv = v4[i];
        const float4 gg = g4[i];
        adam1(pp.x, gg.x, mm.x, vv.x, c, coef);
        adam1(pp.y, gg.y, mm.y, vv.y, c, coef);
        adam1(pp.z, gg.z, mm.z, vv.z, c, coef);
        adam1(pp.w, gg.w, mm.w, vv.w, c, coef);
        p4[i] = pp; m4[i] = mm; v4[i] = vv;
    }
    for (int64_t i = nvec * 4 + tid; i < P; i += nt) adam1(p[i], g[i], m[i], v[i], c, coef);
}

static int adam_step_impl(float *p, const float *g, float *m, float *v, int64_t P, int step, float lr, float beta1,
                          float beta2, float eps, float max_grad_norm, const double *sumsq, float grad_scale,
                          const uint32_t *skip_flag, const float *lr_dev, void *stream, const char *who) {
    SF_REQUIRE(p && g && m && v && P > 0 && step >= 1, "%s: bad args", who);
    SF_REQUIRE((((uintptr_t)p | (uintptr_t)g | (uintptr_t)m | (uintptr_t)v) & 15) == 0,
               "%s: buffers must be 16-byte aligned", who);
    AdamC c;
    const double bc1 = 1.0 - pow((double)beta1, (double)step), bc2 = 1.0 - pow((double)beta2, (double)step);
    c.lr_step = (float)((double)lr / bc1);
    c.bc2_sqrt = (float)sqrt(bc2);
    c.w1 = (float)(1.0 - (double)beta1);
    c.b2 = beta2;
    c.w2 = (float)(1.0 - (double)beta2);
    c.eps = eps;
    c.max_norm = max_grad_norm;
    c.grad_scale = grad_scale;
    const int64_t blocks = (P / 4 + 255) / 256;
    k_adam<<<dim3((unsigned)(blocks < 2048 ? (blocks ? blocks : 1) : 2048)), dim3(256), 0, STREAM(stream)>>>(
        p, g, m, v, P, c, sumsq, skip_flag, lr_dev);
    return sf_launch_status(who);
}

extern "C" int sf_adam_step(float *p, const float *g, float *m, float *v, int64_t P, int step, float lr, float beta1,
                            float beta2, float eps, float max_grad_norm, const double *sumsq, float grad_scale,
                            const uint32_t *skip_flag, void *stream) {
    return adam_step_impl(p, g, m, v, P, step, lr, beta1, beta2, eps, max_grad_norm, sumsq, grad_scale, skip_flag, nullptr,
                          stream, "sf_adam_step");
}
extern "C" int sf_adam_step_dlr(float *p, const float *g, float *m, float *v, int64_t P, int step, const float *lr_dev,
                                float lr_scale, float beta1, float beta2, float eps, float max_grad_norm,
                                const double *sumsq, float grad_scale, const uint32_t *skip_flag, void *stream) {
    SF_REQUIRE(lr_dev, "sf_adam_step_dlr: null lr_dev");
    return adam_step_impl(p, g, m, v, P, step, lr_scale, beta1, beta2, eps, max_grad_norm, sumsq, grad_scale, skip_flag,
                          lr_dev, stream, "sf_adam_step_dlr");
}

__global__ void k_clock_probe(unsigned long long *__restrict__ out, int spin_cycles) {
    if (threadIdx.x || blockIdx.x) return;
    const unsigned long long w0 = wall_clock64(), c0 = clock64();
    unsigned long long c1 = c0;
    while ((long long)(c1 - c0) < (long long)spin_cycles) c1 = clock64();
    const unsigned long long w1 = wall_clock64();
    out[0] = c1 - c0;
    out[1] = w1 - w0;
}
extern "C" int sf_clock_probe(unsigned long long *out, int spin_cycles, void *stream) {
    SF_REQUIRE(out && spin_cycles > 0, "sf_clock_probe: bad args");
    k_clock_probe<<<dim3(1), dim3(64), 0, STREAM(stream)>>>(out, spin_cycles);
    return sf_launch_status("sf_clock_probe");
}

__global__ void k_lr_kl_adaptive(const float *__restrict__ kl, float *__restrict__ lr_dev, float threshold, float lr_min,
                                 float lr_max, float *__restrict__ lr_out) {
    if (threadIdx.x || blockIdx.x) return;
    const double k = (double)*kl;
    double lr = (double)*lr_dev;
    if (k > 2.0 * (double)threshold) lr = fmax(lr / 1.5, (double)lr_min);
    if (k < 0.5 * (double)threshold) lr = fmin(lr * 1.5, (double)lr_max);
    *lr_dev = (float)lr;
    if (lr_out) *lr_out = (float)lr;
}
extern "C" int sf_lr_kl_adaptive(const float *kl, float *lr_dev, float threshold, float lr_min, float lr_max,
                                 float *lr_out, void *stream) {
    SF_REQUIRE(kl && lr_dev, "sf_lr_kl_adaptive: null pointer");
    k_lr_kl_adaptive<<<dim3(1), dim3(64), 0, STREAM(stream)>>>(kl, lr_dev, threshold, lr_min, lr_max, lr_out);
    return sf_launch_status("sf_lr_kl_adaptive");
}

struct LambC {
    float inv_bc1, inv_bc2_sqrt, w1, b1, b2, w2, eps, wd, max_norm, grad_scale, lr, min_trust;
};
constexpr int LAMB_MAX_SEG = 64;

// ... 1151 lines not shown
```

sample_factory_amd/lib.py:

```python
from __future__ import annotations

import ctypes as C
import os
import threading
from typing import Optional

import torch

_HERE = os.path.dirname(os.path.abspath(__file__))
LIB_PATH = os.environ.get("SF_HIP_LIB") or os.path.join(_HERE, "libsf_hip.so")


class SfHipError(RuntimeError):
    pass


class sf_loss_cfg(C.Structure):
    _fields_ = [("clip_ratio", C.c_float), ("clip_value", C.c_float), ("value_loss_coeff", C.c_float),
                ("exploration_coeff", C.c_float), ("kl_coeff", C.c_float), ("exploration_kind", C.c_int32),
                ("action_kind", C.c_int32), ("dense_adv", C.c_int32), ("num_heads", C.c_int32),
                ("head_n", C.c_int32 * 8), ("old_values_T", C.c_int32)]


class sf_conv_desc(C.Structure):
    _fields_ = [("Cin", C.c_int32), ("H", C.c_int32), ("W", C.c_int32), ("Cout", C.c_int32), ("KH", C.c_int32),
                ("KW", C.c_int32), ("stride", C.c_int32), ("OH", C.c_int32), ("OW", C.c_int32),
                ("in_u8", C.c_int32), ("relu", C.c_int32), ("traj_T", C.c_int32), ("sub_mean", C.c_float),
                ("inv_scale", C.c_float)]


IN_F32_NHWC, IN_U8_FRAME, IN_F32_FRAME = 0, 1, 2


class sf_res_desc(C.Structure):
    _fields_ = [("Cin", C.c_int32), ("H", C.c_int32), ("W", C.c_int32), ("Cout", C.c_int32), ("in_u8", C.c_int32),
                ("act_in", C.c_int32), ("traj_T", C.c_int32), ("sub_mean", C.c_float), ("inv_scale", C.c_float)]


SYMBOLS = [
    "sf_last_error", "sf_abi_version", "sf_valid_mask", "sf_gae_returns", "sf_moments", "sf_rms_update",
    "sf_rms_apply", "sf_vtrace", "sf_vtrace_masked", "sf_ppo_loss", "sf_ppo_loss_heads", "sf_ppo_loss_masked", "sf_loss_scalars", "sf_train_summaries", "sf_minibatch_indices", "sf_minibatch_expand", "sf_grad_sumsq",
    "sf_adam_step", "sf_adam_step_dlr", "sf_lr_kl_adaptive", "sf_clock_probe", "sf_lamb_step", "sf_rnn_cell_fwd", "sf_rnn_cell_bwd", "sf_rows_add_scale", "sf_mlp2_fwd", "sf_rnn_store_state", "sf_rnn_chunk_setup", "sf_lstm_seq_supported", "sf_lstm_seq_fwd", "sf_lstm_seq_bwd", "sf_gru_seq_fwd", "sf_gru_seq_bwd", "sf_seq_fwd_x_supported", "sf_lstm_seq_fwd_x", "sf_gru_seq_fwd_x", "sf_rnn_rowseq_supported", "sf_rnn_rowseq_fwd", "sf_rnn_rowseq_bwd", "sf_rnn_wideseq_supported", "sf_rnn_seq_slab_rows", "sf_rnn_wideseq_fwd", "sf_rnn_wideseq_bwd", "sf_linear_fwd_dual_supported", "sf_linear_fwd_dual",
    "sf_obsnorm_moments", "sf_obsnorm_update", "sf_obsnorm_apply", "sf_sample_write_step",
    "sf_sample_write_step_tuple", "sf_sample_write_step_masked", "sf_sample_write_step_tuple_masked",
    "sf_traj_write_env_step", "sf_traj_write_env_step_active", "sf_rnn_store_state_held", "sf_synth_obs",
    "sf_synth_step", "sf_synth_vec_step", "sf_h2d_rows", "sf_copy_rows", "sf_framestack_step", "sf_hwc_to_chw", "sf_framestack_step_hwc", "sf_frame_resize", "sf_conv_fwd", "sf_conv_fwd_workspace", "sf_conv_wgrad_workspace", "sf_conv_wgrad",
    "sf_conv_dgrad", "sf_conv_norm_supported", "sf_conv_fwd_norm", "sf_conv_wgrad_norm", "sf_conv_relu_mask_supported", "sf_conv_fwd_relu_mask", "sf_conv_wgrad_relu_mask", "sf_conv_kernel_name", "sf_conv_fwd_t_supported", "sf_conv_fwd_t_workspace", "sf_conv_fwd_t", "sf_transpose",
    "sf_conv_fwd_os_supported", "sf_conv_fwd_relu_mask_os", "sf_conv_fwd_t_os",
    "sf_conv_fwd_os2_supported", "sf_conv_fwd_relu_mask_os2", "sf_conv_fwd_t_os2",
    "sf_tanh_scale_fwd", "sf_tanh_scale_bwd",
    "sf_linear_fwd", "sf_linear_wgrad_workspace", "sf_linear_wgrad", "sf_linear_dgrad", "sf_relu_mask",
    "sf_dp_unique_id", "sf_dp_comm_create", "sf_dp_comm_destroy", "sf_dp_comm_info", "sf_allreduce_grads",
    "sf_dp_allreduce_f64", "sf_dp_broadcast", "sf_dp_oneshot_create", "sf_dp_oneshot_connect", "sf_dp_oneshot_allreduce_f32",
    "sf_dp_oneshot_allreduce_f64", "sf_dp_oneshot_status", "sf_dp_oneshot_destroy",
    "sf_res_conv_fwd", "sf_res_pool_fwd", "sf_res_pool_bwd", "sf_res_conv_dgrad", "sf_res_conv_wgrad_workspace",
    "sf_res_conv_wgrad", "sf_res_conv_fwd_norm", "sf_res_conv_wgrad_norm",
    "sf_pixcatch_state_words", "sf_pixcatch_reset", "sf_pixcatch_step", "sf_pixcatch_reset_levels",
    "sf_pixcatch_step_levels",
    "sf_random_shift_gather",
    "sf_consistency_loss",
]

_lib: Optional[C.CDLL] = None

_REC = threading.local()
_QUERIES = ("_supported", "_workspace", "_kernel_name", "sf_last_error", "sf_abi_version")
_HOST_STATE = ("sf_h2d_rows", "sf_dp_", "sf_allreduce_grads", "sf_clock_probe")
LAUNCH_PROGRAMS = os.environ.get("SF_LAUNCH_PROGRAMS", "1") != "0"


class LaunchProgram:
    __slots__ = ("calls", "keep", "unsafe")

    def __init__(self):
        self.calls = []
        self.keep = []
        self.unsafe = None

    def replay(self) -> None:
        if PROFILE is None:
            for fn, args, what, _ in self.calls:
                rc = fn(*args)
                if rc:
                    _check(rc, what)
        else:
            for fn, args, what, key in self.calls:
                with _timed(key):
                    _check(fn(*args), what)


class _Recorder:

    def __init__(self, real, prog: LaunchProgram):
        self._real, self.prog, self.key = real, prog, None

    def __getattr__(self, name):
        fn = getattr(self._real, name)
        if name.endswith(_QUERIES):
            return fn
        if name.startswith(_HOST_STATE):
            self.prog.unsafe = self.prog.unsafe or name
            return fn

        def call(*args):
            self.prog.calls.append((fn, args, name, self.key))
            return fn(*args)
        return call


class record_launches:

    def __enter__(self) -> LaunchProgram:
        if getattr(_REC, "rec", None) is not None:
            raise SfHipError("record_launches: already recording on this thread")
        prog = LaunchProgram()
        real = load()
        _REC.rec = _Recorder(real, prog)
        return prog

# ... 512 lines not shown
    else:
        _check(load().sf_ppo_loss(*args, stream()), "sf_ppo_loss")


def consistency_loss(params_t, params_s, ld_params, values_t, values_s, ld_values, valids, index, offset, n, A, action_kind,
                     coeff_policy, coeff_value, mom, sums, g_params_s, g_values_s, head_sizes=None) -> None:
    hn = _head_array(head_sizes) if head_sizes and len(head_sizes) > 1 else None
    key = ("consistency_loss", int(n), int(A)) if _keys_wanted() else None
    with _timed(key):
        _check(load().sf_consistency_loss(_raw(params_t, "f32", "params_t"), _raw(params_s, "f32", "params_s"),
                                          int(ld_params), _raw(values_t, "f32", "values_t"),
                                          _raw(values_s, "f32", "values_s"), int(ld_values), ptr(valids, "u8", "valids"),
                                          ptr(index, "i32", "index"), i64(offset), i64(n), int(A), int(action_kind), hn,
                                          len(head_sizes) if hn is not None else 0, f(coeff_policy), f(coeff_value),
                                          ptr(mom, "f64", "moments"), ptr(sums, "f64", "sums"),
                                          _raw(g_params_s, "f32", "g_params_s"), _raw(g_values_s, "f32", "g_values_s"),
                                          stream()), "sf_consistency_loss")


def loss_scalars(sums, mom, cfg: sf_loss_cfg, out) -> None:
    _check(load().sf_loss_scalars(ptr(sums, "f64"), ptr(mom, "f64"), C.byref(cfg), ptr(out, "f32"), stream()),
           "sf_loss_scalars")


def train_summaries(valids, ratio, values, ld_values, old_values, old_values_T, actions, num_actions, adv, dense_adv,
                    policy_id, policy_version, action_logits, A, index, offset, n, my_policy_id, train_step, clip_ratio,
                    exp_avg_sq, out) -> None:
    _check(load().sf_train_summaries(ptr(valids, "u8", "valids"), ptr(ratio, "f32", "ratio"), _raw(values, "f32", "values"),
                                     int(ld_values), ptr(old_values, "f32", "old_values"), int(old_values_T),
                                     ptr(actions, "f32", "actions"), int(num_actions), ptr(adv, "f32", "adv"),
                                     int(bool(dense_adv)), ptr(policy_id, "i32", "policy_id"),
                                     ptr(policy_version, "f32", "policy_version"), ptr(action_logits, "f32", "action_logits"),
                                     int(A), ptr(index, "i32", "index"), i64(offset), i64(n), int(my_policy_id),
                                     int(train_step), f(clip_ratio), ptr(exp_avg_sq, "f32", "exp_avg_sq"),
                                     i64(exp_avg_sq.numel() if exp_avg_sq is not None else 0), ptr(out, "f64", "out"),
                                     stream()), "sf_train_summaries")


def minibatch_indices(out, experience_size, recurrence, shuffle, seed, epoch) -> None:
    _check(load().sf_minibatch_indices(ptr(out, "i32", "indices"), i64(experience_size), int(recurrence),
                                       int(bool(shuffle)), u32(seed), u32(epoch), stream()), "sf_minibatch_indices")


def minibatch_expand(chunk_starts, out, experience_size, recurrence) -> None:
    _check(load().sf_minibatch_expand(ptr(chunk_starts, "i32", "chunk_starts"), ptr(out, "i32", "out"),
                                      i64(experience_size), int(recurrence), stream()), "sf_minibatch_expand")


def grad_sumsq(g, sumsq) -> None:
    _check(load().sf_grad_sumsq(ptr(g, "f32", "grad"), i64(g.numel()), ptr(sumsq, "f64", "sumsq"), stream()),
           "sf_grad_sumsq")


def adam_step(p, g, m, v, step, lr, beta1, beta2, eps, max_grad_norm, sumsq, grad_scale=1.0, skip_flag=None) -> None:
    _check(load().sf_adam_step(ptr(p, "f32", "params"), ptr(g, "f32", "grads"), ptr(m, "f32", "exp_avg"),
                               ptr(v, "f32", "exp_avg_sq"), i64(p.numel()), int(step), f(lr), f(beta1), f(beta2),
                               f(eps), f(max_grad_norm), ptr(sumsq, "f64", "sumsq"), f(grad_scale),
                               ptr(skip_flag, "i32", "skip_flag"), stream()),
           "sf_adam_step")


def adam_step_dlr(p, g, m, v, step, lr_dev, lr_scale, beta1, beta2, eps, max_grad_norm, sumsq, grad_scale=1.0,
                  skip_flag=None) -> None:
    _check(load().sf_adam_step_dlr(ptr(p, "f32", "params"), ptr(g, "f32", "grads"), ptr(m, "f32", "exp_avg"),
                                   ptr(v, "f32", "exp_avg_sq"), i64(p.numel()), int(step), ptr(lr_dev, "f32", "lr_dev"),
                                   f(lr_scale), f(beta1), f(beta2), f(eps), f(max_grad_norm), ptr(sumsq, "f64", "sumsq"),
                                   f(grad_scale), ptr(skip_flag, "i32", "skip_flag"), stream()), "sf_adam_step_dlr")


def lr_kl_adaptive(kl, lr_dev, threshold, lr_min, lr_max, lr_out=None) -> None:
    _check(load().sf_lr_kl_adaptive(ptr(kl, "f32", "kl"), ptr(lr_dev, "f32", "lr_dev"), f(threshold), f(lr_min), f(lr_max),
                                    ptr(lr_out, "f32", "lr_out"), stream()), "sf_lr_kl_adaptive")


def clock_probe(out: torch.Tensor, spin_cycles: int = 200000, on_stream=None) -> None:
    if not out.is_cuda or out.dtype != torch.int64 or out.numel() < 2:
        raise SfHipError("clock_probe: out must be a device int64 tensor of 2 elements")
    st = C.c_void_p(on_stream.cuda_stream) if on_stream is not None else stream()
    _check(load().sf_clock_probe(C.c_void_p(out.data_ptr()), int(spin_cycles), st), "sf_clock_probe")


def lamb_step(p, g, m, v, scratch, seg_id, seg_sums, num_segments, step, lr, beta1, beta2, eps, weight_decay, min_trust,
              max_grad_norm, sumsq, grad_scale=1.0, skip_flag=None) -> None:
    _check(load().sf_lamb_step(ptr(p, "f32", "p"), ptr(g, "f32", "g"), ptr(m, "f32", "m"), ptr(v, "f32", "v"),
                               ptr(scratch, "f32", "scratch"), ptr(seg_id, "u8", "seg_id"), ptr(seg_sums, "f64", "seg_sums"),
                               i64(p.numel()), int(num_segments), int(step), f(lr), f(beta1), f(beta2), f(eps),
                               f(weight_decay), f(min_trust), f(max_grad_norm), ptr(sumsq, "f64", "sumsq"),
                               f(grad_scale), ptr(skip_flag, "i32", "skip_flag"), stream()), "sf_lamb_step")


def sample_write_step(logits, ld_logits, values, ld_values, B, A, T, t, seed, step, row0, policy_version, deterministic,
                      traj_actions, traj_logits, traj_logp, traj_values, traj_policy_version, env_actions,
                      action_kind=0) -> None:
    _check(load().sf_sample_write_step(_raw(logits, "f32", "logits"), int(ld_logits), _raw(values, "f32", "values"),
                                       int(ld_values), int(B), int(A), int(T),
                                       int(t), u32(seed), u32(step), u32(row0), f(policy_version),
                                       int(bool(deterministic)), int(action_kind), ptr(traj_actions, "f32"),
                                       ptr(traj_logits, "f32"),
                                       ptr(traj_logp, "f32"), ptr(traj_values, "f32"),
                                       ptr(traj_policy_version, "f32"), ptr(env_actions, "i32"), stream()),
           "sf_sample_write_step")


def sample_write_step_masked(logits, ld_logits, values, ld_values, mask, ld_mask, B, A, T, t, seed, step, row0,
                             policy_version, deterministic, traj_actions, traj_logits, traj_logp, traj_values,
                             traj_policy_version, env_actions) -> None:
    if mask.dtype not in (torch.uint8, torch.bool) or not mask.is_cuda:
        raise SfHipError(f"action_mask: expected a u8/bool CUDA tensor, got {mask.dtype} on {mask.device}")
    _check(load().sf_sample_write_step_masked(_raw(logits, "f32", "logits"), int(ld_logits),
                                              _raw(values, "f32", "values"), int(ld_values),
                                              _vp(mask), i64(ld_mask), int(B), int(A), int(T), int(t),
                                              u32(seed), u32(step), u32(row0), f(policy_version),
                                              int(bool(deterministic)), ptr(traj_actions, "f32"),
                                              ptr(traj_logits, "f32"), ptr(traj_logp, "f32"), ptr(traj_values, "f32"),
                                              ptr(traj_policy_version, "f32"), ptr(env_actions, "i32"), stream()),
           "sf_sample_write_step_masked")


def sample_write_step_tuple(logits, ld_logits, values, ld_values, B, head_n, T, t, seed, step, row0, policy_version,
                            deterministic, traj_actions, traj_logits, traj_logp, traj_values, traj_policy_version,
# ... 354 lines not shown

def conv_relu_mask_supported(n, desc: sf_conv_desc) -> bool:
    return bool(load().sf_conv_relu_mask_supported(i64(n), C.byref(desc)))


def conv_fwd_relu_mask(inp, in_sample_stride, index, offset, w, bias, out, relu_mask, n, desc: sf_conv_desc) -> None:
    with _timed(_dkey("fwd", n, desc)):
        _check(load().sf_conv_fwd_relu_mask(_raw_in(inp, desc), i64(in_sample_stride), ptr(index, "i32", "index"),
                                            i64(offset), ptr(w, "f32", "w"), ptr(bias, "f32", "bias"),
                                            ptr(out, "f32", "out"), ptr(relu_mask, "i32", "relu_mask"), i64(n),
                                            C.byref(desc), stream()), "sf_conv_fwd_relu_mask")


def conv_wgrad_relu_mask(inp, in_sample_stride, index, offset, dout, relu_mask, dw, db, n, desc: sf_conv_desc,
                         workspace) -> None:
    with _timed(_dkey("wgrad", n, desc)):
        _check(load().sf_conv_wgrad_relu_mask(_raw_in(inp, desc), i64(in_sample_stride), ptr(index, "i32", "index"),
                                              i64(offset), ptr(dout, "f32", "dout"), ptr(relu_mask, "i32", "relu_mask"),
                                              ptr(dw, "f32", "dw"), ptr(db, "f32", "db"), i64(n), C.byref(desc),
                                              ptr(workspace, "u8", "workspace"), stream()), "sf_conv_wgrad_relu_mask")


def conv_norm_supported(n, desc: sf_conv_desc) -> bool:
    return bool(load().sf_conv_norm_supported(i64(n), C.byref(desc)))


def _nkey(op, n, desc, name_op):
    k = _dkey(op, n, desc)
    if k is None:
        return None
    nk = (name_op,) + k[1:-1] + (desc.in_u8,)
    name = _names.get(nk)
    if name is None:
        name = _names[nk] = conv_kernel_name(_OPS[name_op], n, desc)
    return k[:-1] + (name,)


def conv_fwd_norm(inp, in_sample_stride, index, offset, mu, rstd, w, bias, out, n, desc: sf_conv_desc) -> None:
    with _timed(_nkey("fwd", n, desc, "fwd_norm")):
        _check(load().sf_conv_fwd_norm(_raw_in(inp, desc), i64(in_sample_stride), ptr(index, "i32", "index"), i64(offset),
                                       ptr(mu, "f32", "mu"), ptr(rstd, "f32", "rstd"), ptr(w, "f32", "w"),
                                       ptr(bias, "f32", "bias"), ptr(out, "f32", "out"), i64(n), C.byref(desc),
                                       stream()), "sf_conv_fwd_norm")


def conv_wgrad_norm(inp, in_sample_stride, index, offset, mu, rstd, dout, dw, db, n, desc: sf_conv_desc, workspace) -> None:
    with _timed(_nkey("wgrad", n, desc, "wgrad_norm")):
        _check(load().sf_conv_wgrad_norm(_raw_in(inp, desc), i64(in_sample_stride), ptr(index, "i32", "index"),
                                         i64(offset), ptr(mu, "f32", "mu"), ptr(rstd, "f32", "rstd"),
                                         ptr(dout, "f32", "dout"), ptr(dw, "f32", "dw"), ptr(db, "f32", "db"), i64(n),
                                         C.byref(desc), ptr(workspace, "u8", "workspace"), stream()), "sf_conv_wgrad_norm")


def conv_dgrad(dout, w, in_act, din, n, desc: sf_conv_desc) -> None:
    with _timed(_dkey("dgrad", n, desc)):
        _check(load().sf_conv_dgrad(ptr(dout, "f32", "dout"), ptr(w, "f32", "w"), ptr(in_act, "f32", "in_act"),
                                  ptr(din, "f32", "din"), i64(n), C.byref(desc), stream()), "sf_conv_dgrad")


def conv_fwd_t_supported(n, desc: sf_conv_desc) -> bool:
    return bool(load().sf_conv_fwd_t_supported(i64(n), C.byref(desc)))


def conv_fwd_t_workspace(n, desc: sf_conv_desc) -> int:
    return int(load().sf_conv_fwd_t_workspace(i64(n), C.byref(desc)))


def conv_fwd_t(inp, in_sample_stride, wt, bias, out, n, desc: sf_conv_desc, workspace=None) -> None:
    with _timed(_dkey("fwd_t", n, desc)):
        _check(load().sf_conv_fwd_t(_raw_in(inp, desc), i64(in_sample_stride), ptr(wt, "f32", "wt"),
                                    ptr(bias, "f32", "bias"), ptr(out, "f32", "out"), i64(n), C.byref(desc),
                                    ptr(workspace, "u8", "workspace"),
                                    i64(workspace.numel() if workspace is not None else 0), stream()),
               "sf_conv_fwd_t")


def conv_fwd_os_supported(op: str, n, desc: sf_conv_desc, in_sample_stride, out_sample_stride) -> bool:
    return bool(load().sf_conv_fwd_os_supported(_OPS[op], i64(n), C.byref(desc), i64(in_sample_stride),
                                                i64(out_sample_stride)))


def conv_fwd_relu_mask_os(inp, in_sample_stride, index, offset, w, bias, out, out_sample_stride, relu_mask,
                          mask_sample_stride, n, desc: sf_conv_desc) -> None:
    with _timed(_nkey("fwd", n, desc, "fwd_os")):
        _check(load().sf_conv_fwd_relu_mask_os(_raw_in(inp, desc), i64(in_sample_stride), ptr(index, "i32", "index"),
                                               i64(offset), ptr(w, "f32", "w"), ptr(bias, "f32", "bias"),
                                               _raw(out, "f32", "out"), i64(out_sample_stride),
                                               _raw(relu_mask, "i32", "relu_mask"), i64(mask_sample_stride), i64(n),
                                               C.byref(desc), stream()), "sf_conv_fwd_relu_mask_os")


def conv_fwd_t_os(inp, in_sample_stride, wt, bias, out, out_sample_stride, n, desc: sf_conv_desc) -> None:
    with _timed(_nkey("fwd_t", n, desc, "fwd_t_os")):
        _check(load().sf_conv_fwd_t_os(_raw_in(inp, desc), i64(in_sample_stride), ptr(wt, "f32", "wt"),
                                       ptr(bias, "f32", "bias"), _raw(out, "f32", "out"), i64(out_sample_stride), i64(n),
                                       C.byref(desc), stream()), "sf_conv_fwd_t_os")


def _raw_opt(t, kind, name):
    return _raw(t, kind, name) if t is not None else C.c_void_p(0)


def conv_fwd_os2_supported(op: str, n, keep_n, desc: sf_conv_desc, in_sample_stride, out_sample_stride) -> bool:
    return bool(load().sf_conv_fwd_os2_supported(_OPS[op], i64(n), i64(keep_n), C.byref(desc), i64(in_sample_stride),
                                                 i64(out_sample_stride)))

# ... 204 lines not shown
```

sample_factory_amd/model/actor_critic.py:

```python
from __future__ import annotations

import math
import threading
from typing import Dict, List, Optional

import numpy as np
import torch

from sample_factory_amd import lib
from sample_factory_amd.algo.learning.rollout_reuse import SlotRecord, fc_reusable, keep_n, keep_rows, reuse_prefix, twin_name
from sample_factory_amd.algo.utils.running_mean_std import RunningMeanStdInPlace
from sample_factory_amd.envs.spaces import is_box, calc_num_action_parameters

import os

_LSTM_SEQ = os.environ.get("SF_LSTM_SEQ", "1") != "0"
_CONV1_NORM = os.environ.get("SF_CONV1_NORM", "1") != "0"
_MLP2 = os.environ.get("SF_MLP2", "1") != "0"
_REUSE = os.environ.get("SF_REUSE_ROLLOUT_ACTS", "1") != "0"
KEEP_MEM_SHARE = 0.5

ACT_KIND = {"relu": 1, "tanh": 2, "elu": 3}
FRAME_KINDS = {"conv_u8": lib.IN_U8_FRAME, "conv_f32frame": lib.IN_F32_FRAME}

# ... 39 lines not shown
    def out_pixels(self):
        return self.desc.OH * self.desc.OW

    def w_from_ref(self, w_ref: torch.Tensor) -> torch.Tensor:
        d = self.desc
        if self.kind in FRAME_KINDS:
            return w_ref.reshape(d.Cout, self.K).t().contiguous()
        if self.kind == "conv":
            return w_ref.permute(2, 3, 1, 0).reshape(self.K, d.Cout).contiguous()
        if self.kind == "linear_after_conv":
            C, OH, OW = self.first_fc_chw
            return w_ref.view(self.N, C, OH, OW).permute(2, 3, 1, 0).reshape(self.K, self.N).contiguous()
        return w_ref.t().contiguous()

    def w_to_ref(self, w: torch.Tensor) -> torch.Tensor:
        d = self.desc
        if self.kind in FRAME_KINDS:
            return w.t().reshape(d.Cout, d.Cin, d.KH, d.KW).contiguous()
        if self.kind == "conv":
            return w.reshape(d.KH, d.KW, d.Cin, d.Cout).permute(3, 2, 0, 1).contiguous()
        if self.kind == "linear_after_conv":
            C, OH, OW = self.first_fc_chw
            return w.reshape(OH, OW, C, self.N).permute(3, 2, 0, 1).reshape(self.N, self.K).contiguous()
        return w.t().contiguous()


def _linear_desc(K, N, relu) -> lib.sf_conv_desc:
    return lib.sf_conv_desc(Cin=K, H=1, W=1, Cout=N, KH=1, KW=1, stride=1, OH=1, OW=1, in_u8=0, relu=int(relu),
                            traj_T=0, sub_mean=0.0, inv_scale=1.0)


class NativeModel:

    def eval(self):
        return self.train(False)

    def model_to_device(self, device):
        assert torch.device(device).type == "cuda", "the native model only lives on the GPU"

    def normalize_obs(self, obs):
        return obs


class NativeTower(NativeModel):

    def _init_scratch(self) -> None:
        self._bufs: Dict = {}
        self._layout_gen = 0
        self._wss: Dict = {}
        self._tls = threading.local()
        self._snap = None
        self._snap_tabs = None
        self.snap_read = 0

    def _buf(self, key, shape, dtype=torch.float32):
        t = self._bufs.get(key)
        if t is None or t.shape != torch.Size(shape) or t.dtype != dtype:
            t = torch.empty(shape, dtype=dtype, device=self.device)
            self._bufs[key] = t
            self._layout_gen += 1
        return t

    def _zbuf(self, key, shape):
        t = self._bufs.get(key)
        if t is None or t.shape != torch.Size(shape):
            t = torch.zeros(shape, dtype=torch.float32, device=self.device)
            self._bufs[key] = t
            self._layout_gen += 1
        return t

    def _workspace(self, nbytes: int) -> torch.Tensor:
        key = getattr(self._tls, "role", "learner")
        ws = self._wss.get(key)
        if ws is None or ws.numel() < nbytes:
            ws = torch.empty(max(int(nbytes), 16), dtype=torch.uint8, device=self.device)
            self._wss[key] = ws
            self._layout_gen += 1
        return ws

    def launch_key(self, tag: str = "inf"):
        return (self._layout_gen, self.snap_read if self._snap is not None else -1)

    @property
    def _norm_prefix(self) -> str:
        return f"obs_normalizer.running_mean_std.running_mean_std.{self.obs_key}."

    def normalizer_state(self) -> Dict[str, torch.Tensor]:
        return self.obs_normalizer.state_dict(self._norm_prefix) if self.obs_normalizer is not None else {}

    def load_normalizer_state(self, sd) -> None:
        if self.obs_normalizer is not None and self._norm_prefix + "count" in sd:
            self.obs_normalizer.load_state_dict(sd, self._norm_prefix)

    def initialize_weights(self):
        cfg = self.cfg
        gain = cfg.policy_init_gain
        sd = {}
        for name, shape in self.ref_param_shapes():
            t = torch.empty(shape, dtype=torch.float32)
            if name.endswith("learned_stddev"):
                t.fill_(math.log(cfg.initial_stddev))
            elif name.startswith("core.core."):
                bound = 1.0 / math.sqrt(self.rnn_H)
                t.uniform_(-bound, bound)
            elif name.endswith(".bias"):
                if cfg.policy_initialization == "torch_default":
                    fan_in = int(np.prod(dict(self.ref_param_shapes())[name[:-4] + "weight"][1:]))
                    bound = 1 / math.sqrt(fan_in)
                    t.uniform_(-bound, bound)
                else:
                    t.zero_()
            elif cfg.policy_initialization == "orthogonal":
                torch.nn.init.orthogonal_(t, gain=gain)
            elif cfg.policy_initialization == "xavier_uniform":
                torch.nn.init.xavier_uniform_(t, gain=gain)
            else:
                torch.nn.init.kaiming_uniform_(t, a=math.sqrt(5))
            sd[name] = t
        self.load_state_dict(sd, strict=False)


class ActorCritic(NativeTower):

    def __init__(self, cfg, obs_space, action_space, device="cuda", all_reduce=None, obs_key: str = "obs", part: str = "full"):
        assert part in ("full", "encoder", "trunk")
# ... 266 lines not shown
            return out
        H, (o, ob), A = self.layers[-1], self._segs[-1], self.num_action_params
        w = flat[o:o + H.K * H.N].view(H.K, H.N).cpu()
        b = flat[ob:ob + H.N].cpu()
        out["critic_linear.weight"] = w[:, 0:1].t().contiguous()
        out["critic_linear.bias"] = b[0:1].clone()
        Aw = A // 2 if self.nonadaptive_std else A
        out["action_parameterization.distribution_linear.weight"] = w[:, 1:1 + Aw].t().contiguous()
        out["action_parameterization.distribution_linear.bias"] = b[1:1 + Aw].clone()
        if self.nonadaptive_std:
            out["action_parameterization.learned_stddev"] = b[1 + Aw:1 + A].clone()
        return out

    def _aligned_frames(self, tag, x, stride, idx, off, tT, n):
        d = idx.long() if idx is not None else torch.arange(off, off + n, device=x.device)
        pos = d + torch.div(d, int(tT), rounding_mode="floor") if tT else d
        avail = (x.untyped_storage().nbytes() - x.storage_offset() * x.element_size()) // x.element_size()
        rows = (avail - self.obs_elems) // int(stride) + 1
        flat = x.as_strided((rows, self.obs_elems), (int(stride), 1))
        out = self._buf((tag, "frames_aligned"), (n, self.obs_elems), dtype=x.dtype)
        lib.recording_unsafe("frames gathered by a torch op")
        torch.index_select(flat, 0, pos, out=out)
        return out, self.obs_elems, None, 0, 0

    def _frames_vector_geometry(self) -> bool:
        d = self.layers[0].desc
        return d.KW % 4 == 0 and d.stride % 4 == 0 and d.W % 4 == 0

    def tensor_segment_ids(self):
        seg = torch.full((self.num_flat,), 255, dtype=torch.uint8)
        nseg = 0
        for L, (o, ob) in zip(self._body(), self._segs):
            seg[o:o + L.K * L.N] = nseg
            seg[ob:ob + L.N] = nseg + 1
            nseg += 2
        if self.headless:
            return seg.to(self.device), nseg
        H, (o, ob), A = self.layers[-1], self._segs[-1], self.num_action_params
        hw = torch.full((H.K, H.N), 255, dtype=torch.uint8)
        hw[:, 0] = nseg
        Aw = A // 2 if self.nonadaptive_std else A
        hw[:, 1:1 + Aw] = nseg + 2
        seg[o:o + H.K * H.N] = hw.reshape(-1)
        hb = torch.full((H.N,), 255, dtype=torch.uint8)
        hb[0] = nseg + 1
        hb[1:1 + Aw] = nseg + 3
        if self.nonadaptive_std:
            hb[1 + Aw:1 + A] = nseg + 4
        seg[ob:ob + H.N] = hb
        return seg.to(self.device), nseg + (5 if self.nonadaptive_std else 4)

    def params_changed(self) -> None:
        self.weights_gen += 1
        for L in self.layers:
            if L.wt is not None:
                lib.transpose(L.w, L.wt, L.K, L.N)

    def enable_weight_snapshots(self) -> None:
        self._snap = [self.flat_params.clone(), self.flat_params.clone()]
        self._snap_t = [self.flat_params_t.clone(), self.flat_params_t.clone()]
        self._snap_views = []
        for buf, buft in zip(self._snap, self._snap_t):
            self._snap_views.append([(buf[o:o + L.K * L.N].view(L.K, L.N), buf[ob:ob + L.N],
                                      buft[o:o + L.K * L.N].view(L.N, L.K) if L.wt is not None else None)
                                     for L, (o, ob) in zip(self.layers, self._segs)])
        self.snap_read = 0
        self._layout_gen += 1
        on = self.obs_normalizer
        self._snap_tabs = [(on.mu_tab.clone(), on.rstd_tab.clone()) for _ in range(2)] if on is not None else None

    def publish_weights(self, slot: int) -> None:
        self.weights_gen += 1
        self._snap[slot].copy_(self.flat_params)
        self._snap_t[slot].copy_(self.flat_params_t)
        if self._snap_tabs is not None:
            self._snap_tabs[slot][0].copy_(self.obs_normalizer.mu_tab)
            self._snap_tabs[slot][1].copy_(self.obs_normalizer.rstd_tab)

    def _wb(self, li, tag):
        if tag.startswith("inf") and self._snap is not None:
            return self._snap_views[self.snap_read][li]
        L = self.layers[li]
        return L.w, L.b, L.wt

    def _gemm(self, li, x, stride, index, offset, traj_T, out, n, tag):
        L = self.layers[li]
        d = L.desc
        if traj_T:
            d = lib.sf_conv_desc.from_buffer_copy(L.desc)
            d.traj_T = int(traj_T)
        w, b, wt = self._wb(li, tag)
        if wt is not None and index is None and not traj_T and lib.conv_fwd_t_supported(n, d):
            wsb = lib.conv_fwd_t_workspace(n, d)
            lib.conv_fwd_t(x, stride, wt, b, out, n, d, self._workspace(wsb) if wsb else None)
            return
        wsb = lib.conv_fwd_workspace(n, d) if index is None and not traj_T else 0
        lib.conv_fwd_raw(x, stride, index, offset, w, b, out, n, d, self._workspace(wsb) if wsb else None)

    def forward_heads(self, obs: torch.Tensor, n: int, *, sample_stride: int, index=None, offset: int = 0,
                      traj_T: int = 0, tag="inf", rnn=None, keep=None, resume_from=None) -> List[torch.Tensor]:
        acts: List[Optional[torch.Tensor]] = [None] * len(self.layers)
        inputs: List[Optional[torch.Tensor]] = [None] * len(self.layers)
        relu_mask0 = None
        self._tls.role = "rollout" + tag[3:] if tag.startswith("inf") else "learner"
        x, stride, idx, off, tT = obs, sample_stride, index, offset, traj_T
        first_layer = 0
# ... 399 lines not shown
        lib.conv_wgrad_raw(sv["Hprev"][:R].reshape(n, H), H, None, 0, dGH.view(n, GH), Lh.gw, Lh.gb, n, Lh.desc, ws)
        return dGX.view(n, GH)

    def new_rnn_parts_of(self, tag: str = "inf"):
        return self._rnn_out.get(tag)

    def new_rnn_states_of(self, tag: str = "inf") -> torch.Tensor:
        return torch.cat([t for h, c in self._rnn_out[tag] for t in ((h,) if c is None else (h, c))], dim=1)

    @property
    def new_rnn_states(self) -> torch.Tensor:
        return self.new_rnn_states_of("inf")

    def _seq_sync_buf(self) -> torch.Tensor:
        t = self._bufs.get(("rnn", "seq_sync"))
        if t is None:
            t = self._bufs[("rnn", "seq_sync")] = torch.zeros(192, dtype=torch.int32, device=self.device)
        return t

    def rnn_abort_word(self) -> Optional[torch.Tensor]:
        return self._seq_sync_buf()[128:129] if (self.rnn_kind is not None and _LSTM_SEQ) else None

    def rnn_abort_clear(self) -> None:
        if self.rnn_kind is not None and _LSTM_SEQ:
            self._seq_sync_buf()[128:129].zero_()

    def rnn_pass_aborted(self) -> bool:
        t = self._bufs.get(("rnn", "seq_sync"))
        return t is not None and bool(int(t[128].item()))

    def forward(self, normalized_obs_dict, rnn_states=None, values_only: bool = False, action_mask=None):
        obs = normalized_obs_dict["obs"] if isinstance(normalized_obs_dict, dict) else normalized_obs_dict
        B = obs.shape[0]
        rnn = dict(states=rnn_states) if self.rnn_kind is not None else None
        heads = self.forward_heads(obs, B, sample_stride=self.obs_elems if obs.is_contiguous() else obs.stride(0),
                                   rnn=rnn)[-1]
        res = dict(values=heads[:, 0])
        if not values_only:
            res["action_logits"] = heads[:, 1:1 + self.num_action_params]
        res["new_rnn_states"] = self.new_rnn_states if self.rnn_kind is not None else rnn_states
        return res

    def backward(self, acts: List[torch.Tensor], g_heads: torch.Tensor, obs: torch.Tensor, n: int, *,
                 sample_stride: int, index=None, offset: int = 0, traj_T: int = 0, on_layer_done=None) -> None:
        ctx = self._ctx["train"]
        self._tls.role = "learner"
        inputs = ctx["inputs"]
        x0, stride0, idx0, off0, tT0 = ctx["first_in"]
        g = g_heads
        if self.tanh_scale > 0:
            lib.tanh_scale_bwd(g_heads, ctx["acts"][-1], self.heads_ld, n, 1, self.num_action_params // 2, self.tanh_scale)
        chain = [li for li, L in enumerate(self.layers) if L.role != "rnn_hh"]
        mask0 = ctx.get("relu_mask0")
        for pos in range(len(chain) - 1, -1, -1):
            li = chain[pos]
            L = self.layers[li]
            d = L.desc
            if L.role == "rnn_ih":
                g = self._rnn_sequence_bwd(li, g, n)
            if pos == 0 and not self.features_in:
                d0 = lib.sf_conv_desc.from_buffer_copy(d)
                d0.traj_T = int(tT0)
                ws = self._workspace(lib.conv_wgrad_workspace(n, d0))
                if ctx.get("norm_tabs") is not None:
                    mu_, rstd_ = ctx["norm_tabs"]
                    lib.conv_wgrad_norm(x0, stride0, idx0, off0, mu_, rstd_, g, L.gw, L.gb, n, d0, ws)
                elif mask0 is not None:
                    lib.conv_wgrad_relu_mask(x0, stride0, idx0, off0, g, mask0, L.gw, L.gb, n, d0, ws)
                else:
                    lib.conv_wgrad_raw(x0, stride0, idx0, off0, g, L.gw, L.gb, n, d0, ws)
            else:
                x = inputs[li]
                ws = self._workspace(lib.conv_wgrad_workspace(n, d))
                lib.conv_wgrad_raw(x, d.H * d.W * d.Cin, None, 0, g, L.gw, L.gb, n, d, ws)
                gin = self._buf(("g", li - 1), tuple(x.shape))
                dd = lib.sf_conv_desc.from_buffer_copy(d)
                dd.relu = L.in_act_kind
                if pos == 1 and mask0 is not None:
                    dd.relu = 0
                    lib.conv_dgrad(g, L.w, None, gin, n, dd)
                else:
                    lib.conv_dgrad(g, L.w, x if L.in_act_kind else None, gin, n, dd)
                g = gin
                if L.role == "rnn_ih":
                    R, Cn = self._rnn_saved["R"], self._rnn_saved["Cn"]
                    gs = self._buf(("g", "x_sm", li), (n, L.K))
                    gs.view(Cn, R, L.K).copy_(g.view(R, Cn, L.K).transpose(0, 1))
                    g = gs
                if pos == 0:
                    self.g_input = g
            if self.nonadaptive_std and li == len(self.layers) - 1:
                A = self.num_action_params
                L.gw[:, 1 + A // 2:1 + A].zero_()
            if on_layer_done is not None:
                on_layer_done(li)
```

Measured before the change: 2.247 million.

## Fold wgrad reductions, weight transposes and invalid count into batched device launches

Wgrad partial reductions for all layers are deferred and run as one multi-segment kernel driven by a device-side segment table. Per-layer weight transposes after each step are likewise batched into one launch. The invalid-sample count is no longer read back with a blocking .item() before training: it is passed into a new Adam kernel and read back with the first epoch's stats. This cuts launch count and host-device syncs, at the cost of per-layer workspaces, more complex control flow, and possibly rolling back steps when every sample is invalid.

```diff
diff --git a/include/sf_hip.h b/include/sf_hip.h
--- a/include/sf_hip.h
+++ b/include/sf_hip.h
@@ -111,6 +111,9 @@
 int sf_adam_step_dlr(float *p, const float *g, float *m, float *v, int64_t P, int step, const float *lr_dev,
                      float lr_scale, float beta1, float beta2, float eps, float max_grad_norm, const double *sumsq,
                      float grad_scale, const uint32_t *skip_flag, void *stream);
+int sf_adam_step_ninv(float *p, const float *g, float *m, float *v, int64_t P, int step, double lr, const float *lr_dev,
+                      const int32_t *num_invalid, int64_t size, int32_t *count_out, float beta1, float beta2, float eps,
+                      float max_grad_norm, const double *sumsq, float grad_scale, const uint32_t *skip_flag, void *stream);
 int sf_lr_kl_adaptive(const float *kl, float *lr_dev, float threshold, float lr_min, float lr_max, float *lr_out,
                       void *stream);
 int sf_clock_probe(unsigned long long *out, int spin_cycles, void *stream);
@@ -229,6 +232,15 @@
 int sf_conv_wgrad_norm(const void *in, int64_t in_sample_stride, const int32_t *index, int64_t offset, const float *mu,
                        const float *rstd, const float *dout, float *dw, float *db, int64_t n, const sf_conv_desc *h_desc,
                        void *workspace, void *stream);
+
+int sf_step_fold_enabled(void);
+int sf_conv_wgrad_partials(const void *in, int64_t in_sample_stride, const int32_t *index, int64_t offset, const float *mu,
+                           const float *rstd, const float *dout, const uint32_t *relu_mask, float *dw, float *db,
+                           int64_t n, const sf_conv_desc *h_desc, void *workspace, int64_t *h_segs, void *stream);
+int sf_reduce_partials(const float *partial, float *out, int64_t n, int Z, void *stream);
+int sf_reduce_plan(int64_t n, int Z, int64_t *h_tree_blocks);
+int sf_reduce_partials_multi(const void *table, int nsegs, int64_t total_blocks, void *stream);
+int sf_transpose_multi(const void *table, int nsegs, int64_t total_blocks, void *stream);
 
 int sf_mlp2_fwd(const float *x, int64_t x_stride, int64_t n, int D, float sub_mean, float inv_scale, const float *mu,
                 const float *rstd, const float *w1, const float *b1, int H1, const float *w2, const float *b2, int H2,
diff --git a/sample_factory_amd/algo/learning/learner.py b/sample_factory_amd/algo/learning/learner.py
--- a/sample_factory_amd/algo/learning/learner.py
+++ b/sample_factory_amd/algo/learning/learner.py
@@ -384,7 +384,7 @@
         self.policy_versions_tensor[self.policy_id] = self.train_step
         self.policy_to_load = None
 
-    def _prepare_batch(self, batch: TensorDict) -> Tuple[AttrDict, int, int]:
+    def _prepare_batch(self, batch: TensorDict, defer_count: bool = False) -> Tuple[AttrDict, int, int]:
         cfg, ac = self.cfg, self.actor_critic
         multi = getattr(ac, "multi_key", False)
         obs = {k: batch["obs"][k] for k in ac.obs_keys} if multi else batch["obs"]["obs"]
@@ -429,6 +429,9 @@
             buff.action_mask = batch["obs"]["action_mask"]
         if cfg.normalize_returns and not cfg.with_vtrace:
             ac.returns_normalizer(buff.returns)
+        if defer_count:
+            self._global_invalids = None
+            return buff, N, None
         num_invalids = int(self._num_invalid.item())
         if self.dp:
             t = torch.tensor([num_invalids], dtype=torch.int64, device=self.device)
@@ -437,6 +440,9 @@
         else:
             self._global_invalids = num_invalids
         return buff, N, num_invalids
+
+    def _count_on_device(self) -> bool:
+        return not self.dp and self.cfg.optimizer == "adam" and lib.step_fold_enabled()
 
     def _get_minibatches(self, batch_size, experience_size):
         cfg = self.cfg
@@ -580,7 +586,12 @@
         recent_kls: List[float] = []
         num_sgd_steps = 0
         n_mb = cfg.num_batches_per_epoch
-        self._scalars = ac._buf(("loss", "scalars"), (cfg.num_epochs * n_mb, 16))
+        sbuf = ac._buf(("loss", "scalars"), (1 + cfg.num_epochs * n_mb, 16))
+        self._scalars = sbuf[1:]
+        count_dev = self._global_invalids is None
+        count_out = sbuf[0, :1].view(torch.int32) if count_dev else None
+        ninv = dict(num_invalid=self._num_invalid, size=experience_size * self.world, count_out=count_out) if count_dev else {}
+        steps0 = (self.adam_step_count, self.train_step)
         global_size = experience_size * self.world
         need_kl_each_mb = self.lr_scheduler.invoke_after_each_minibatch() and isinstance(self.lr_scheduler, KlAdaptiveScheduler)
         self._dp_reduce_each_mb = need_kl_each_mb
@@ -619,7 +630,7 @@
                         self.group.all_reduce_grads(ac.flat_grads)
                 actual_lr = self.curr_lr
                 valid_frac = 1.0
-                if self._global_invalids > 0:
+                if self._global_invalids is not None and self._global_invalids > 0:
                     valid_frac = (global_size - self._global_invalids) / global_size
                     actual_lr = self.curr_lr * valid_frac
                 self.adam_step_count += 1
@@ -642,12 +653,12 @@
                     lib.adam_step_dlr(ac.flat_params, ac.flat_grads, self.exp_avg, self.exp_avg_sq, self.adam_step_count,
                                       self._lr_dev, valid_frac, cfg.adam_beta1, cfg.adam_beta2, cfg.adam_eps,
                                       cfg.max_grad_norm if use_clip else 0.0, self._sumsq if use_clip else None,
-                                      skip_flag=skip)
+                                      skip_flag=skip, **ninv)
                 else:
                     lib.adam_step(ac.flat_params, ac.flat_grads, self.exp_avg, self.exp_avg_sq, self.adam_step_count,
-                                  actual_lr, cfg.adam_beta1, cfg.adam_beta2, cfg.adam_eps,
+                                  self.curr_lr if count_dev else actual_lr, cfg.adam_beta1, cfg.adam_beta2, cfg.adam_eps,
                                   cfg.max_grad_norm if use_clip else 0.0, self._sumsq if use_clip else None,
-                                  skip_flag=skip)
+                                  skip_flag=skip, **ninv)
                 ac.params_changed()
                 num_sgd_steps += 1
                 self.train_step += 1
@@ -671,7 +682,19 @@
                 aborted = bool(self.group.all_reduce_max(skip.to(torch.float32)).item() != 0)
             else:
                 aborted = skip is not None and ac.rnn_pass_aborted()
-            rows = blk.cpu()
+            if count_dev and epoch == 0:
+                rows = sbuf[:1 + n_mb].cpu()
+                self._global_invalids = int(rows[0, :1].view(torch.int32)[0])
+                rows = rows[1:]
+                if self._global_invalids >= global_size:
+                    self.adam_step_count, self.train_step = steps0
+                    self.policy_versions_tensor[self.policy_id] = self.train_step
+                    return None
+                if self._global_invalids > 0:
+                    valid_frac = (global_size - self._global_invalids) / global_size
+                    actual_lr = actual_lr * valid_frac
+            else:
+                rows = blk.cpu()
             if aborted:
                 raise lib.SfHipError(
                     "a fused recurrent sequence pass was aborted (a work-group never arrived: is the GPU shared with "
@@ -736,10 +759,12 @@
     def train(self, batch: TensorDict) -> Optional[Dict]:
         self._maybe_update_cfg()
         self._maybe_load_policy()
-        buff, experience_size, num_invalids = self._prepare_batch(batch)
-        if self._global_invalids >= experience_size * self.world:
+        buff, experience_size, num_invalids = self._prepare_batch(batch, defer_count=self._count_on_device())
+        if self._global_invalids is not None and self._global_invalids >= experience_size * self.world:
             return None
         train_stats = self._train(buff, self.cfg.batch_size, experience_size, num_invalids)
+        if train_stats is None and self._global_invalids is not None and self._global_invalids >= experience_size * self.world:
+            return None
         frameskip = self.env_info.frameskip if self.cfg.summaries_use_frameskip else 1
         self.env_steps += experience_size * self.world * frameskip
         stats = {LEARNER_ENV_STEPS: self.env_steps, POLICY_ID_KEY: self.policy_id}
diff --git a/sample_factory_amd/csrc/sf_nn.hip b/sample_factory_amd/csrc/sf_nn.hip
--- a/sample_factory_amd/csrc/sf_nn.hip
+++ b/sample_factory_amd/csrc/sf_nn.hip
@@ -630,9 +630,9 @@
         }
 }
 
-__global__ __launch_bounds__(256) void k_reduce_partials(const float *__restrict__ partial, float *__restrict__ out,
-                                                         int64_t n, int Z) {
-    for (int64_t i = (int64_t)blockIdx.x * blockDim.x + threadIdx.x; i < n; i += (int64_t)gridDim.x * blockDim.x) {
+__device__ __forceinline__ void reduce_plain(const float *__restrict__ partial, float *__restrict__ out, int64_t n, int Z,
+                                             int64_t block, int64_t nblocks) {
+    for (int64_t i = block * blockDim.x + threadIdx.x; i < n; i += nblocks * blockDim.x) {
         float s[8] = {0.f, 0.f, 0.f, 0.f, 0.f, 0.f, 0.f, 0.f};
         int z = 0;
         for (; z + 8 <= Z; z += 8) {
@@ -643,12 +643,16 @@
         out[i] = ((s[0] + s[1]) + (s[2] + s[3])) + ((s[4] + s[5]) + (s[6] + s[7]));
     }
 }
-
-__global__ __launch_bounds__(256) void k_reduce_partials_tree(const float *__restrict__ partial, float *__restrict__ out,
-                                                              int64_t n, int Z) {
+__global__ __launch_bounds__(256) void k_reduce_partials(const float *__restrict__ partial, float *__restrict__ out,
+                                                         int64_t n, int Z) {
+    reduce_plain(partial, out, n, Z, blockIdx.x, gridDim.x);
+}
+
+__device__ __forceinline__ void reduce_tree(const float *__restrict__ partial, float *__restrict__ out, int64_t n, int Z,
+                                            int64_t block) {
     __shared__ float sm[8][33];
     const int li = threadIdx.x & 31, zg = threadIdx.x >> 5;
-    const int64_t i = (int64_t)blockIdx.x * 32 + li;
+    const int64_t i = block * 32 + li;
     const int zper = (Z + 7) / 8, z0 = zg * zper, z1 = z0 + zper < Z ? z0 + zper : Z;
     float s[8] = {0.f, 0.f, 0.f, 0.f, 0.f, 0.f, 0.f, 0.f};
     if (i < n) {
@@ -663,6 +667,33 @@
     __syncthreads();
     if (zg == 0 && i < n)
         out[i] = ((sm[0][li] + sm[1][li]) + (sm[2][li] + sm[3][li])) + ((sm[4][li] + sm[5][li]) + (sm[6][li] + sm[7][li]));
+}
+__global__ __launch_bounds__(256) void k_reduce_partials_tree(const float *__restrict__ partial, float *__restrict__ out,
+                                                              int64_t n, int Z) {
+    reduce_tree(partial, out, n, Z, blockIdx.x);
+}
+struct ReduceSeg {
+    const float *src;
+    float *dst;
+    int64_t n, Z, tree, block0, blocks, pad;
+};
+struct ReducePair { ReduceSeg s[2]; };
+__device__ __forceinline__ void reduce_seg(const ReduceSeg &g, int64_t b) {
+    const int64_t lb = b - g.block0;
+    if (lb < 0 || lb >= g.blocks) return;
+    if (g.tree) reduce_tree(g.src, g.dst, g.n, (int)g.Z, lb);
+    else reduce_plain(g.src, g.dst, g.n, (int)g.Z, lb, g.blocks);
+}
+__global__ __launch_bounds__(256) void k_reduce_partials_pair(ReducePair p) {
+    const ReduceSeg g = blockIdx.x >= p.s[1].block0 ? p.s[1] : p.s[0];
+    reduce_seg(g, blockIdx.x);
+}
+__global__ __launch_bounds__(256) void k_reduce_partials_multi(const ReduceSeg *__restrict__ segs, int nsegs) {
+    const int64_t b = blockIdx.x;
+    int s = 0;
+    while (s + 1 < nsegs && b >= segs[s + 1].block0) ++s;
+    const ReduceSeg g = segs[s];
+    reduce_seg(g, b);
 }
 #define SF_SWITCHES(X)                                                                                                  \
     X(reduce_tree, "SF_REDUCE_TREE", 1) X(conv1_bf16, "SF_CONV1_BF16", 1) X(conv1_img, "SF_CONV1_IMG", 1)              \
@@ -676,7 +707,8 @@
     X(tap_perm, "SF_TAP_PERM", 0) X(wgrad_glds, "SF_WGRAD_GLDS", 1) X(wgrad_glds_min, "SF_WGRAD_GLDS_MIN", -1)         \
     X(wgrad_glds_k64, "SF_WGRAD_GLDS_K64", 1) X(wgrad_img, "SF_WGRAD_IMG", 3) X(wgrad_zl, "SF_WGRAD_ZL", 1)            \
     X(dgrad_linear, "SF_DGRAD_LINEAR", 1) X(dgrad_linear64, "SF_DGRAD_LINEAR64", 1) X(dgrad_lpt, "SF_DGRAD_LPT", 1)    \
-    X(dgrad_zl, "SF_DGRAD_ZL", 3) X(dgrad_pix, "SF_DGRAD_PIX", 1) X(debug_occ, "SF_DEBUG_OCC", 0)
+    X(dgrad_zl, "SF_DGRAD_ZL", 3) X(dgrad_pix, "SF_DGRAD_PIX", 1) X(debug_occ, "SF_DEBUG_OCC", 0)                      \
+    X(step_fold, "SF_STEP_FOLD", 1)
 struct Switches {
 #define X(field, name, dflt) int64_t field;
     SF_SWITCHES(X)
@@ -700,11 +732,56 @@
     return s;
 }
 
+static ReduceSeg plan_reduce(const float *partial, float *out, int64_t n, int Z) {
+    ReduceSeg r = {partial, out, n, Z, 0, 0, 0, 0};
+    r.tree = sw().reduce_tree && Z >= 64 && (n + 255) / 256 < 256;
+    r.blocks = r.tree ? (n + 31) / 32 : ((n + 255) / 256 < 2048 ? (n + 255) / 256 : 2048);
+    return r;
+}
 static void launch_reduce_partials(const float *partial, float *out, int64_t n, int Z, hipStream_t st) {
-    if (sw().reduce_tree && Z >= 64 && (n + 255) / 256 < 256)
-        k_reduce_partials_tree<<<dim3((unsigned)((n + 31) / 32)), dim3(256), 0, st>>>(partial, out, n, Z);
-    else
-        k_reduce_partials<<<dim3((unsigned)((n + 255) / 256 < 2048 ? (n + 255) / 256 : 2048)), dim3(256), 0, st>>>(partial, out, n, Z);
+    const ReduceSeg r = plan_reduce(partial, out, n, Z);
+    if (r.tree) k_reduce_partials_tree<<<dim3((unsigned)r.blocks), dim3(256), 0, st>>>(partial, out, n, Z);
+    else k_reduce_partials<<<dim3((unsigned)r.blocks), dim3(256), 0, st>>>(partial, out, n, Z);
+}
+static void finish_wgrad(const float *partial_w, float *dw, int64_t KN, const float *partial_b, float *db, int N, int Z,
+                         hipStream_t st, int64_t *defer) {
+    ReducePair p;
+    p.s[0] = plan_reduce(partial_w, dw, KN, Z);
+    p.s[1] = db ? plan_reduce(partial_b, db, N, Z) : ReduceSeg{nullptr, nullptr, 0, 0, 0, 0, 0, 0};
+    p.s[1].block0 = p.s[0].blocks;
+    if (defer) {
+        for (int i = 0; i < 2; ++i) {
+            const ReduceSeg &r = p.s[i];
+            int64_t *o = defer + 8 * i;
+            o[0] = (int64_t)(uintptr_t)r.src; o[1] = (int64_t)(uintptr_t)r.dst; o[2] = r.n; o[3] = r.Z; o[4] = r.tree;
+            o[5] = 0; o[6] = r.blocks; o[7] = 0;
+        }
+    } else if (sw().step_fold && db) {
+        k_reduce_partials_pair<<<dim3((unsigned)(p.s[0].blocks + p.s[1].blocks)), dim3(256), 0, st>>>(p);
+    } else {
+        launch_reduce_partials(partial_w, dw, KN, Z, st);
+        if (db) launch_reduce_partials(partial_b, db, N, Z, st);
+    }
+}
+extern "C" int sf_step_fold_enabled(void) { return sw().step_fold != 0; }
+extern "C" int sf_reduce_partials(const float *partial, float *out, int64_t n, int Z, void *stream) {
+    SF_REQUIRE(partial && out && n > 0 && Z > 0, "sf_reduce_partials: bad args");
+    launch_reduce_partials(partial, out, n, Z, STREAM(stream));
+    return sf_launch_status("sf_reduce_partials");
+}
+extern "C" int sf_reduce_plan(int64_t n, int Z, int64_t *h_tree_blocks) {
+    SF_REQUIRE(h_tree_blocks && n > 0 && Z > 0, "sf_reduce_plan: bad args");
+    const ReduceSeg r = plan_reduce(nullptr, nullptr, n, Z);
+    h_tree_blocks[0] = r.tree; h_tree_blocks[1] = r.blocks;
+    return SF_OK;
+}
+extern "C" int sf_reduce_partials_multi(const void *table, int nsegs, int64_t total_blocks, void *stream) {
+    SF_REQUIRE(nsegs >= 0 && total_blocks >= 0 && total_blocks < (1LL << 31), "sf_reduce_partials_multi: bad args");
+    if (nsegs == 0 || total_blocks == 0) return SF_OK;
+    SF_REQUIRE(table && ((uintptr_t)table & 7) == 0, "sf_reduce_partials_multi: table must be an 8-byte aligned device buffer");
+    k_reduce_partials_multi<<<dim3((unsigned)total_blocks), dim3(256), 0, STREAM(stream)>>>(
+        reinterpret_cast<const ReduceSeg *>(table), nsegs);
+    return sf_launch_status("sf_reduce_partials_multi");
 }
 
 template <int BM, int BN, int WM, int WN, bool VEC>
@@ -1498,6 +1575,14 @@
     SF_REQUIRE(w && wt && K > 0 && N > 0, "sf_transpose: bad args");
     k_transpose<<<dim3(cdiv64(K, 32), cdiv64(N, 32)), dim3(256), 0, STREAM(stream)>>>(w, wt, K, N);
     return sf_launch_status("sf_transpose");
+}
+extern "C" int sf_transpose_multi(const void *table, int nsegs, int64_t total_blocks, void *stream) {
+    SF_REQUIRE(nsegs >= 0 && total_blocks >= 0 && total_blocks < (1LL << 31), "sf_transpose_multi: bad args");
+    if (nsegs == 0 || total_blocks == 0) return SF_OK;
+    SF_REQUIRE(table && ((uintptr_t)table & 7) == 0, "sf_transpose_multi: table must be an 8-byte aligned device buffer");
+    k_transpose_multi<<<dim3((unsigned)total_blocks), dim3(256), 0, STREAM(stream)>>>(
+        reinterpret_cast<const TransposeSeg *>(table), nsegs);
+    return sf_launch_status("sf_transpose_multi");
 }
 
 struct SplitPlan {
@@ -1673,7 +1758,7 @@
 static int conv_wgrad_impl(const void *in, int64_t in_sample_stride, const int32_t *index, int64_t offset,
                            const float *dout, const uint32_t *dmask, float *dw, float *db, int64_t n,
                            const sf_conv_desc *h_desc, void *workspace, void *stream, const float *mu = nullptr,
-                           const float *rstd = nullptr) {
+                           const float *rstd = nullptr, int64_t *defer = nullptr) {
     int rc = check_desc(h_desc, "sf_conv_wgrad");
     if (rc) return rc;
     SF_REQUIRE(in && dout && dw && workspace && n > 0, "sf_conv_wgrad: bad args");
@@ -1715,8 +1800,7 @@
             if (TILE_IS(128, 32)) { BY_MODE(WGRAD_LAUNCH, 32, 4, 1) }
             else { BY_MODE(WGRAD_LAUNCH, 64, 2, 2) }
     }
-    launch_reduce_partials(partial_w, dw, (int64_t)K * N, p.partials, st);
-    if (db) launch_reduce_partials(partial_b, db, N, p.partials, st);
+    finish_wgrad(partial_w, dw, (int64_t)K * N, partial_b, db, N, p.partials, st, defer);
     return sf_launch_status("sf_conv_wgrad");
 }
 
@@ -1758,9 +1842,9 @@
         g, reinterpret_cast<const uint8_t *>(in), in_sample_stride, index, offset, w, bias, out, (int)n);
     return sf_launch_status("sf_conv_fwd_norm");
 }
-extern "C" int sf_conv_wgrad_norm(const void *in, int64_t in_sample_stride, const int32_t *index, int64_t offset,
-                                  const float *mu, const float *rstd, const float *dout, float *dw, float *db, int64_t n,
-                                  const sf_conv_desc *h_desc, void *workspace, void *stream) {
+static int conv_wgrad_norm_impl(const void *in, int64_t in_sample_stride, const int32_t *index, int64_t offset,
+                                const float *mu, const float *rstd, const float *dout, float *dw, float *db, int64_t n,
+                                const sf_conv_desc *h_desc, void *workspace, void *stream, int64_t *defer) {
     int rc = check_desc(h_desc, "sf_conv_wgrad_norm");
     if (rc) return rc;
     SF_REQUIRE(in && mu && rstd && dout && dw && workspace && n > 0, "sf_conv_wgrad_norm: bad args");
@@ -1772,15 +1856,37 @@
     const ConvPlan p = plan_conv_wgrad(h_desc, g, n, Operands{in, in_sample_stride, index != nullptr, nullptr, dout, nullptr, 0});
     if (p.kernel != K_CONV1_WGRAD_IMG_NORM)
         return conv_wgrad_impl(in, in_sample_stride, index, offset, dout, nullptr, dw, db, n, h_desc, workspace, stream, mu,
-                               rstd);
+                               rstd, defer);
     SF_REQUIRE(((uintptr_t)workspace & 15) == 0, "sf_conv_wgrad_norm: workspace must be 16-byte aligned");
     const int K = g.K, N = g.Cout;
     float *partial_w = reinterpret_cast<float *>(workspace), *partial_b = db ? partial_w + (int64_t)p.partials * K * N : nullptr;
     hipStream_t st = STREAM(stream);
     WGRAD_STRIP((k_conv1_wgrad_img_norm<2, 4>));
-    launch_reduce_partials(partial_w, dw, (int64_t)K * N, p.partials, st);
-    if (db) launch_reduce_partials(partial_b, db, N, p.partials, st);
+    finish_wgrad(partial_w, dw, (int64_t)K * N, partial_b, db, N, p.partials, st, defer);
     return sf_launch_status("sf_conv_wgrad_norm");
+}
+extern "C" int sf_conv_wgrad_norm(const void *in, int64_t in_sample_stride, const int32_t *index, int64_t offset,
+                                  const float *mu, const float *rstd, const float *dout, float *dw, float *db, int64_t n,
+                                  const sf_conv_desc *h_desc, void *workspace, void *stream) {
+    return conv_wgrad_norm_impl(in, in_sample_stride, index, offset, mu, rstd, dout, dw, db, n, h_desc, workspace, stream,
+                                nullptr);
+}
+extern "C" int sf_conv_wgrad_partials(const void *in, int64_t in_sample_stride, const int32_t *index, int64_t offset,
+                                      const float *mu, const float *rstd, const float *dout, const uint32_t *relu_mask,
+                                      float *dw, float *db, int64_t n, const sf_conv_desc *h_desc, void *workspace,
+                                      int64_t *h_segs, void *stream) {
+    SF_REQUIRE(h_segs && (mu != nullptr) == (rstd != nullptr) && !(mu && relu_mask), "sf_conv_wgrad_partials: bad args");
+    if (mu)
+        return conv_wgrad_norm_impl(in, in_sample_stride, index, offset, mu, rstd, dout, dw, db, n, h_desc, workspace, stream,
+                                    h_segs);
+    if (relu_mask) {
+        SF_REQUIRE(((uintptr_t)relu_mask & 7) == 0, "sf_conv_wgrad_partials: relu_mask must be an 8-byte aligned device buffer");
+        SF_REQUIRE(h_desc && n > 0 && relu_mask_ok(h_desc, n) && ((uintptr_t)in & 3) == 0 && in_sample_stride % 4 == 0 &&
+                       ((uintptr_t)dout & 15) == 0,
+                   "sf_conv_wgrad_partials: unsupported layer / launch (see sf_conv_relu_mask_supported)");
+    }
+    return conv_wgrad_impl(in, in_sample_stride, index, offset, dout, relu_mask, dw, db, n, h_desc, workspace, stream, nullptr,
+                           nullptr, h_segs);
 }
 
 static sf_conv_desc linear_desc(int K, int N, int relu);
diff --git a/sample_factory_amd/csrc/sf_nn_glds.h b/sample_factory_amd/csrc/sf_nn_glds.h
--- a/sample_factory_amd/csrc/sf_nn_glds.h
+++ b/sample_factory_amd/csrc/sf_nn_glds.h
@@ -687,9 +687,10 @@
     }
 }
 
-__global__ __launch_bounds__(256) void k_transpose(const float *__restrict__ w, float *__restrict__ wt, int K, int N) {
+__device__ __forceinline__ void transpose_tile(const float *__restrict__ w, float *__restrict__ wt, int K, int N, int bx,
+                                               int by) {
     __shared__ float t[32][33];
-    const int k0 = blockIdx.x * 32, n0 = blockIdx.y * 32, tx = threadIdx.x & 31, ty = threadIdx.x >> 5;
+    const int k0 = bx * 32, n0 = by * 32, tx = threadIdx.x & 31, ty = threadIdx.x >> 5;
 #pragma unroll
     for (int i = 0; i < 32; i += 8) {
         const int k = k0 + ty + i, n = n0 + tx;
@@ -701,6 +702,23 @@
         const int n = n0 + ty + i, k = k0 + tx;
         if (n < N && k < K) wt[(int64_t)n * K + k] = t[tx][ty + i];
     }
+}
+__global__ __launch_bounds__(256) void k_transpose(const float *__restrict__ w, float *__restrict__ wt, int K, int N) {
+    transpose_tile(w, wt, K, N, blockIdx.x, blockIdx.y);
+}
+struct TransposeSeg {
+    const float *w;
+    float *wt;
+    int64_t K, N, nbx, block0, blocks, pad;
+};
+__global__ __launch_bounds__(256) void k_transpose_multi(const TransposeSeg *__restrict__ segs, int nsegs) {
+    const int64_t b = blockIdx.x;
+    int s = 0;
+    while (s + 1 < nsegs && b >= segs[s + 1].block0) ++s;
+    const TransposeSeg g = segs[s];
+    const int64_t lb = b - g.block0;
+    if (lb < 0 || lb >= g.blocks) return;
+    transpose_tile(g.w, g.wt, (int)g.K, (int)g.N, (int)(lb % g.nbx), (int)(lb / g.nbx));
 }
 
 __device__ __attribute__((aligned(128))) const float sf_zero_page[32] = {};
diff --git a/sample_factory_amd/csrc/sf_rl.hip b/sample_factory_amd/csrc/sf_rl.hip
--- a/sample_factory_amd/csrc/sf_rl.hip
+++ b/sample_factory_amd/csrc/sf_rl.hip
@@ -2032,12 +2032,9 @@
     p = p - c.lr_step * (m / denom);
 }
 
-__global__ __launch_bounds__(256) void k_adam(float *__restrict__ p, const float *__restrict__ g,
-                                              float *__restrict__ m, float *__restrict__ v, int64_t P, AdamC c,
-                                              const double *__restrict__ sumsq, const uint32_t *__restrict__ skip,
-                                              const float *__restrict__ lr_dev) {
-    if (skip && *skip) return;
-    if (lr_dev) c.lr_step *= *lr_dev;
+__device__ __forceinline__ void adam_body(float *__restrict__ p, const float *__restrict__ g, float *__restrict__ m,
+                                          float *__restrict__ v, int64_t P, const AdamC &c,
+                                          const double *__restrict__ sumsq) {
     float coef = c.grad_scale;
     if (sumsq && c.max_norm > 0.f) {
         const float total = (float)sqrt(*sumsq) * fabsf(c.grad_scale);
@@ -2059,10 +2056,36 @@
     }
     for (int64_t i = nvec * 4 + tid; i < P; i += nt) adam1(p[i], g[i], m[i], v[i], c, coef);
 }
+__global__ __launch_bounds__(256) void k_adam(float *__restrict__ p, const float *__restrict__ g,
+                                              float *__restrict__ m, float *__restrict__ v, int64_t P, AdamC c,
+                                              const double *__restrict__ sumsq, const uint32_t *__restrict__ skip,
+                                              const float *__restrict__ lr_dev) {
+    if (skip && *skip) return;
+    if (lr_dev) c.lr_step *= *lr_dev;
+    adam_body(p, g, m, v, P, c, sumsq);
+}
+__global__ __launch_bounds__(256) void k_adam_ninv(float *__restrict__ p, const float *__restrict__ g,
+                                                   float *__restrict__ m, float *__restrict__ v, int64_t P, AdamC c,
+                                                   const double *__restrict__ sumsq, const uint32_t *__restrict__ skip,
+                                                   const float *__restrict__ lr_dev, const int32_t *__restrict__ num_invalid,
+                                                   int64_t size, double lr_base, double bc1,
+                                                   int32_t *__restrict__ count_out) {
+    const int64_t inv = *num_invalid;
+    if (count_out && blockIdx.x == 0 && threadIdx.x == 0) *count_out = (int32_t)inv;
+    if (skip && *skip) return;
+    if (inv >= size) return;
+    double a = lr_base;
+    if (inv > 0) a = lr_base * ((double)(size - inv) / (double)size);
+    c.lr_step = (float)((double)(float)a / bc1);
+    if (lr_dev) c.lr_step *= *lr_dev;
+    adam_body(p, g, m, v, P, c, sumsq);
+}
 
 static int adam_step_impl(float *p, const float *g, float *m, float *v, int64_t P, int step, float lr, float beta1,
                           float beta2, float eps, float max_grad_norm, const double *sumsq, float grad_scale,
-                          const uint32_t *skip_flag, const float *lr_dev, void *stream, const char *who) {
+                          const uint32_t *skip_flag, const float *lr_dev, void *stream, const char *who,
+                          const int32_t *num_invalid = nullptr, int64_t size = 0, double lr_base = 0.0,
+                          int32_t *count_out = nullptr) {
     SF_REQUIRE(p && g && m && v && P > 0 && step >= 1, "%s: bad args", who);
     SF_REQUIRE((((uintptr_t)p | (uintptr_t)g | (uintptr_t)m | (uintptr_t)v) & 15) == 0,
                "%s: buffers must be 16-byte aligned", who);
@@ -2077,9 +2100,21 @@
     c.max_norm = max_grad_norm;
     c.grad_scale = grad_scale;
     const int64_t blocks = (P / 4 + 255) / 256;
-    k_adam<<<dim3((unsigned)(blocks < 2048 ? (blocks ? blocks : 1) : 2048)), dim3(256), 0, STREAM(stream)>>>(
-        p, g, m, v, P, c, sumsq, skip_flag, lr_dev);
+    const dim3 grid((unsigned)(blocks < 2048 ? (blocks ? blocks : 1) : 2048));
+    if (num_invalid)
+        k_adam_ninv<<<grid, dim3(256), 0, STREAM(stream)>>>(p, g, m, v, P, c, sumsq, skip_flag, lr_dev, num_invalid, size,
+                                                            lr_base, bc1, count_out);
+    else
+        k_adam<<<grid, dim3(256), 0, STREAM(stream)>>>(p, g, m, v, P, c, sumsq, skip_flag, lr_dev);
     return sf_launch_status(who);
+}
+extern "C" int sf_adam_step_ninv(float *p, const float *g, float *m, float *v, int64_t P, int step, double lr,
+                                 const float *lr_dev, const int32_t *num_invalid, int64_t size, int32_t *count_out,
+                                 float beta1, float beta2, float eps, float max_grad_norm, const double *sumsq,
+                                 float grad_scale, const uint32_t *skip_flag, void *stream) {
+    SF_REQUIRE(num_invalid && size > 0, "sf_adam_step_ninv: bad args");
+    return adam_step_impl(p, g, m, v, P, step, 0.f, beta1, beta2, eps, max_grad_norm, sumsq, grad_scale, skip_flag, lr_dev,
+                          stream, "sf_adam_step_ninv", num_invalid, size, lr, count_out);
 }
 
 extern "C" int sf_adam_step(float *p, const float *g, float *m, float *v, int64_t P, int step, float lr, float beta1,
diff --git a/sample_factory_amd/lib.py b/sample_factory_amd/lib.py
--- a/sample_factory_amd/lib.py
+++ b/sample_factory_amd/lib.py
@@ -40,12 +40,14 @@
 SYMBOLS = [
     "sf_last_error", "sf_abi_version", "sf_valid_mask", "sf_gae_returns", "sf_moments", "sf_rms_update",
     "sf_rms_apply", "sf_vtrace", "sf_vtrace_masked", "sf_ppo_loss", "sf_ppo_loss_heads", "sf_ppo_loss_masked", "sf_loss_scalars", "sf_train_summaries", "sf_minibatch_indices", "sf_minibatch_expand", "sf_grad_sumsq",
-    "sf_adam_step", "sf_adam_step_dlr", "sf_lr_kl_adaptive", "sf_clock_probe", "sf_lamb_step", "sf_rnn_cell_fwd", "sf_rnn_cell_bwd", "sf_rows_add_scale", "sf_mlp2_fwd", "sf_rnn_store_state", "sf_rnn_chunk_setup", "sf_lstm_seq_supported", "sf_lstm_seq_fwd", "sf_lstm_seq_bwd", "sf_gru_seq_fwd", "sf_gru_seq_bwd", "sf_seq_fwd_x_supported", "sf_lstm_seq_fwd_x", "sf_gru_seq_fwd_x", "sf_rnn_rowseq_supported", "sf_rnn_rowseq_fwd", "sf_rnn_rowseq_bwd", "sf_rnn_wideseq_supported", "sf_rnn_seq_slab_rows", "sf_rnn_wideseq_fwd", "sf_rnn_wideseq_bwd", "sf_linear_fwd_dual_supported", "sf_linear_fwd_dual",
+    "sf_adam_step", "sf_adam_step_dlr", "sf_adam_step_ninv", "sf_lr_kl_adaptive", "sf_clock_probe", "sf_lamb_step", "sf_rnn_cell_fwd", "sf_rnn_cell_bwd", "sf_rows_add_scale", "sf_mlp2_fwd", "sf_rnn_store_state", "sf_rnn_chunk_setup", "sf_lstm_seq_supported", "sf_lstm_seq_fwd", "sf_lstm_seq_bwd", "sf_gru_seq_fwd", "sf_gru_seq_bwd", "sf_seq_fwd_x_supported", "sf_lstm_seq_fwd_x", "sf_gru_seq_fwd_x", "sf_rnn_rowseq_supported", "sf_rnn_rowseq_fwd", "sf_rnn_rowseq_bwd", "sf_rnn_wideseq_supported", "sf_rnn_seq_slab_rows", "sf_rnn_wideseq_fwd", "sf_rnn_wideseq_bwd", "sf_linear_fwd_dual_supported", "sf_linear_fwd_dual",
     "sf_obsnorm_moments", "sf_obsnorm_update", "sf_obsnorm_apply", "sf_sample_write_step",
     "sf_sample_write_step_tuple", "sf_sample_write_step_masked", "sf_sample_write_step_tuple_masked",
     "sf_traj_write_env_step", "sf_traj_write_env_step_active", "sf_rnn_store_state_held", "sf_synth_obs",
     "sf_synth_step", "sf_synth_vec_step", "sf_h2d_rows", "sf_copy_rows", "sf_framestack_step", "sf_hwc_to_chw", "sf_framestack_step_hwc", "sf_frame_resize", "sf_conv_fwd", "sf_conv_fwd_workspace", "sf_conv_wgrad_workspace", "sf_conv_wgrad",
     "sf_conv_dgrad", "sf_conv_norm_supported", "sf_conv_fwd_norm", "sf_conv_wgrad_norm", "sf_conv_relu_mask_supported", "sf_conv_fwd_relu_mask", "sf_conv_wgrad_relu_mask", "sf_conv_kernel_name", "sf_conv_fwd_t_supported", "sf_conv_fwd_t_workspace", "sf_conv_fwd_t", "sf_transpose",
+    "sf_step_fold_enabled", "sf_conv_wgrad_partials", "sf_reduce_partials", "sf_reduce_plan", "sf_reduce_partials_multi",
+    "sf_transpose_multi",
     "sf_conv_fwd_os_supported", "sf_conv_fwd_relu_mask_os", "sf_conv_fwd_t_os",
     "sf_conv_fwd_os2_supported", "sf_conv_fwd_relu_mask_os2", "sf_conv_fwd_t_os2",
     "sf_tanh_scale_fwd", "sf_tanh_scale_bwd",
@@ -64,7 +66,7 @@
 _lib: Optional[C.CDLL] = None
 
 _REC = threading.local()
-_QUERIES = ("_supported", "_workspace", "_kernel_name", "sf_last_error", "sf_abi_version")
+_QUERIES = ("_supported", "_workspace", "_kernel_name", "sf_last_error", "sf_abi_version", "_enabled", "sf_reduce_plan")
 _HOST_STATE = ("sf_h2d_rows", "sf_dp_", "sf_allreduce_grads", "sf_clock_probe")
 LAUNCH_PROGRAMS = os.environ.get("SF_LAUNCH_PROGRAMS", "1") != "0"
 
@@ -683,7 +685,11 @@
            "sf_grad_sumsq")
 
 
-def adam_step(p, g, m, v, step, lr, beta1, beta2, eps, max_grad_norm, sumsq, grad_scale=1.0, skip_flag=None) -> None:
+def adam_step(p, g, m, v, step, lr, beta1, beta2, eps, max_grad_norm, sumsq, grad_scale=1.0, skip_flag=None, *,
+              num_invalid=None, size=0, count_out=None) -> None:
+    if num_invalid is not None:
+        return adam_step_ninv(p, g, m, v, step, lr, None, num_invalid, size, count_out, beta1, beta2, eps, max_grad_norm,
+                              sumsq, grad_scale, skip_flag)
     _check(load().sf_adam_step(ptr(p, "f32", "params"), ptr(g, "f32", "grads"), ptr(m, "f32", "exp_avg"),
                                ptr(v, "f32", "exp_avg_sq"), i64(p.numel()), int(step), f(lr), f(beta1), f(beta2),
                                f(eps), f(max_grad_norm), ptr(sumsq, "f64", "sumsq"), f(grad_scale),
@@ -692,11 +698,24 @@
 
 
 def adam_step_dlr(p, g, m, v, step, lr_dev, lr_scale, beta1, beta2, eps, max_grad_norm, sumsq, grad_scale=1.0,
-                  skip_flag=None) -> None:
+                  skip_flag=None, *, num_invalid=None, size=0, count_out=None) -> None:
+    if num_invalid is not None:
+        return adam_step_ninv(p, g, m, v, step, 1.0, lr_dev, num_invalid, size, count_out, beta1, beta2, eps, max_grad_norm,
+                              sumsq, grad_scale, skip_flag)
     _check(load().sf_adam_step_dlr(ptr(p, "f32", "params"), ptr(g, "f32", "grads"), ptr(m, "f32", "exp_avg"),
                                    ptr(v, "f32", "exp_avg_sq"), i64(p.numel()), int(step), ptr(lr_dev, "f32", "lr_dev"),
                                    f(lr_scale), f(beta1), f(beta2), f(eps), f(max_grad_norm), ptr(sumsq, "f64", "sumsq"),
                                    f(grad_scale), ptr(skip_flag, "i32", "skip_flag"), stream()), "sf_adam_step_dlr")
+
+
+def adam_step_ninv(p, g, m, v, step, lr, lr_dev, num_invalid, size, count_out, beta1, beta2, eps, max_grad_norm, sumsq,
+                   grad_scale=1.0, skip_flag=None) -> None:
+    _check(load().sf_adam_step_ninv(ptr(p, "f32", "params"), ptr(g, "f32", "grads"), ptr(m, "f32", "exp_avg"),
+                                    ptr(v, "f32", "exp_avg_sq"), i64(p.numel()), int(step), C.c_double(float(lr)),
+                                    ptr(lr_dev, "f32", "lr_dev"), ptr(num_invalid, "i32", "num_invalid"), i64(size),
+                                    ptr(count_out, "i32", "count_out"), f(beta1), f(beta2), f(eps), f(max_grad_norm),
+                                    ptr(sumsq, "f64", "sumsq"), f(grad_scale), ptr(skip_flag, "i32", "skip_flag"),
+                                    stream()), "sf_adam_step_ninv")
 
 
 def lr_kl_adaptive(kl, lr_dev, threshold, lr_min, lr_max, lr_out=None) -> None:
@@ -1157,6 +1176,83 @@
                                          C.byref(desc), ptr(workspace, "u8", "workspace"), stream()), "sf_conv_wgrad_norm")
 
 
+def step_fold_enabled() -> bool:
+    return bool(load().sf_step_fold_enabled())
+
+
+def conv_wgrad_partials(inp, in_sample_stride, index, offset, dout, dw, db, n, desc: sf_conv_desc, workspace, *,
+                        mu=None, rstd=None, relu_mask=None) -> list:
+    segs = (C.c_int64 * 16)()
+    key = _nkey("wgrad", n, desc, "wgrad_norm") if mu is not None else _dkey("wgrad", n, desc)
+    with _timed(key):
+        _check(load().sf_conv_wgrad_partials(_raw_in(inp, desc), i64(in_sample_stride), ptr(index, "i32", "index"),
+                                             i64(offset), ptr(mu, "f32", "mu"), ptr(rstd, "f32", "rstd"),
+                                             ptr(dout, "f32", "dout"), ptr(relu_mask, "i32", "relu_mask"),
+                                             ptr(dw, "f32", "dw"), ptr(db, "f32", "db"), i64(n), C.byref(desc),
+                                             ptr(workspace, "u8", "workspace"), segs, stream()), "sf_conv_wgrad_partials")
+    return [list(segs[8 * i:8 * i + 8]) for i in range(2) if segs[8 * i + 2] > 0]
+
+
+def reduce_plan(n: int, Z: int):
+    out = (C.c_int64 * 2)()
+    _check(load().sf_reduce_plan(i64(n), int(Z), out), "sf_reduce_plan")
+    return int(out[0]), int(out[1])
+
+
+def reduce_segment(partial, out, n: int, Z: int) -> list:
+    tree, blocks = reduce_plan(n, Z)
+    return [ptr(partial, "f32", "partial").value or 0, ptr(out, "f32", "out").value or 0, int(n), int(Z), tree, 0, blocks, 0]
+
+
+def table_rows(segs, first=5, count=6):
+    rows, total = [], 0
+    for r in segs:
+        if r[count] <= 0:
+            continue
+        r = list(r)
+        r[first] = total
+        total += r[count]
+        rows.append(r)
+    return rows, total
+
+
+def transpose_segment_rows(shapes):
+    return [[w, wt, K, N, (K + 31) // 32, 0, ((K + 31) // 32) * ((N + 31) // 32), 0] for w, wt, K, N in shapes]
+
+
+class SegTable:
+
+    def __init__(self):
+        self.rows, self.total, self.dev, self._seen = [], 0, None, {}
+
+    def set(self, segs, device) -> "SegTable":
+        rows, total = table_rows(segs)
+        if rows != self.rows or self.dev is None:
+            key = tuple(map(tuple, rows))
+            dev = self._seen.get(key)
+            if dev is None and rows:
+                if len(self._seen) >= 16:
+                    self._seen.clear()
+                dev = self._seen[key] = torch.tensor(rows, dtype=torch.int64).reshape(-1, 8).to(device)
+            self.rows, self.total, self.dev = rows, total, dev
+        return self
+
+
+def reduce_partials(partial, out, n: int, Z: int) -> None:
+    _check(load().sf_reduce_partials(ptr(partial, "f32", "partial"), ptr(out, "f32", "out"), i64(n), int(Z), stream()),
+           "sf_reduce_partials")
+
+
+def reduce_partials_multi(table: SegTable) -> None:
+    _check(load().sf_reduce_partials_multi(_vp(table.dev) if table.dev is not None else C.c_void_p(0), len(table.rows),
+                                           i64(table.total), stream()), "sf_reduce_partials_multi")
+
+
+def transpose_multi(table: SegTable) -> None:
+    _check(load().sf_transpose_multi(_vp(table.dev) if table.dev is not None else C.c_void_p(0), len(table.rows),
+                                     i64(table.total), stream()), "sf_transpose_multi")
+
+
 def conv_dgrad(dout, w, in_act, din, n, desc: sf_conv_desc) -> None:
     with _timed(_dkey("dgrad", n, desc)):
         _check(load().sf_conv_dgrad(ptr(dout, "f32", "dout"), ptr(w, "f32", "w"), ptr(in_act, "f32", "in_act"),
diff --git a/sample_factory_amd/model/actor_critic.py b/sample_factory_amd/model/actor_critic.py
--- a/sample_factory_amd/model/actor_critic.py
+++ b/sample_factory_amd/model/actor_critic.py
@@ -115,6 +115,7 @@
         self._snap = None
         self._snap_tabs = None
         self.snap_read = 0
+        self._wgrad_table, self._wt_table = lib.SegTable(), lib.SegTable()
 
     def _buf(self, key, shape, dtype=torch.float32):
         t = self._bufs.get(key)
@@ -134,6 +135,15 @@
 
     def _workspace(self, nbytes: int) -> torch.Tensor:
         key = getattr(self._tls, "role", "learner")
+        ws = self._wss.get(key)
+        if ws is None or ws.numel() < nbytes:
+            ws = torch.empty(max(int(nbytes), 16), dtype=torch.uint8, device=self.device)
+            self._wss[key] = ws
+            self._layout_gen += 1
+        return ws
+
+    def _workspace_layer(self, li: int, nbytes: int) -> torch.Tensor:
+        key = ("wgrad", li)
         ws = self._wss.get(key)
         if ws is None or ws.numel() < nbytes:
             ws = torch.empty(max(int(nbytes), 16), dtype=torch.uint8, device=self.device)
@@ -506,6 +516,11 @@
 
     def params_changed(self) -> None:
         self.weights_gen += 1
+        if lib.step_fold_enabled():
+            rows = lib.transpose_segment_rows([(L.w.data_ptr(), L.wt.data_ptr(), L.K, L.N) for L in self.layers
+                                               if L.wt is not None])
+            lib.transpose_multi(self._wt_table.set(rows, self.device))
+            return
         for L in self.layers:
             if L.wt is not None:
                 lib.transpose(L.w, L.wt, L.K, L.N)
@@ -1011,6 +1026,8 @@
             lib.tanh_scale_bwd(g_heads, ctx["acts"][-1], self.heads_ld, n, 1, self.num_action_params // 2, self.tanh_scale)
         chain = [li for li, L in enumerate(self.layers) if L.role != "rnn_hh"]
         mask0 = ctx.get("relu_mask0")
+        fold = on_layer_done is None and lib.step_fold_enabled()
+        segs = []
         for pos in range(len(chain) - 1, -1, -1):
             li = chain[pos]
             L = self.layers[li]
@@ -1020,6 +1037,12 @@
             if pos == 0 and not self.features_in:
                 d0 = lib.sf_conv_desc.from_buffer_copy(d)
                 d0.traj_T = int(tT0)
+                if fold:
+                    ws = self._workspace_layer(li, lib.conv_wgrad_workspace(n, d0))
+                    mu_, rstd_ = ctx["norm_tabs"] if ctx.get("norm_tabs") is not None else (None, None)
+                    segs += lib.conv_wgrad_partials(x0, stride0, idx0, off0, g, L.gw, L.gb, n, d0, ws, mu=mu_, rstd=rstd_,
+                                                    relu_mask=mask0 if mu_ is None else None)
+                    continue
                 ws = self._workspace(lib.conv_wgrad_workspace(n, d0))
                 if ctx.get("norm_tabs") is not None:
                     mu_, rstd_ = ctx["norm_tabs"]
@@ -1030,8 +1053,12 @@
                     lib.conv_wgrad_raw(x0, stride0, idx0, off0, g, L.gw, L.gb, n, d0, ws)
             else:
                 x = inputs[li]
-                ws = self._workspace(lib.conv_wgrad_workspace(n, d))
-                lib.conv_wgrad_raw(x, d.H * d.W * d.Cin, None, 0, g, L.gw, L.gb, n, d, ws)
+                if fold:
+                    ws = self._workspace_layer(li, lib.conv_wgrad_workspace(n, d))
+                    segs += lib.conv_wgrad_partials(x, d.H * d.W * d.Cin, None, 0, g, L.gw, L.gb, n, d, ws)
+                else:
+                    ws = self._workspace(lib.conv_wgrad_workspace(n, d))
+                    lib.conv_wgrad_raw(x, d.H * d.W * d.Cin, None, 0, g, L.gw, L.gb, n, d, ws)
                 gin = self._buf(("g", li - 1), tuple(x.shape))
                 dd = lib.sf_conv_desc.from_buffer_copy(d)
                 dd.relu = L.in_act_kind
@@ -1048,8 +1075,13 @@
                     g = gs
                 if pos == 0:
                     self.g_input = g
-            if self.nonadaptive_std and li == len(self.layers) - 1:
+            if self.nonadaptive_std and li == len(self.layers) - 1 and not fold:
                 A = self.num_action_params
                 L.gw[:, 1 + A // 2:1 + A].zero_()
             if on_layer_done is not None:
                 on_layer_done(li)
+        if fold:
+            lib.reduce_partials_multi(self._wgrad_table.set(segs, self.device))
+            if self.nonadaptive_std:
+                A = self.num_action_params
+                self.layers[-1].gw[:, 1 + A // 2:1 + A].zero_()
```

After: 2.252 million, median of 3. About the same (+0.2%).
